# OpenRL-Lab/openrl

Measured on NVIDIA H100. Metric: env-steps/sec (collect+update), CartPole-v1 PPO, higher is better.
Workload: dtype f32 (nets, losses, Adam; the three 64x64 GEMM groups of the update run as split-fp16 wgmma MMAs with fp32 accumulation = fp32-class accuracy, the mode the 1e-4 parity tests run in), f64 (CartPole state)

## Files before the change

### include/openrl_b200.h

```cpp
#ifndef OPENRL_B200_H
#define OPENRL_B200_H

#include <stdint.h>

#ifdef __cplusplus
extern "C" {
#endif

#define ORL_ABI_VERSION 1

#define ORL_ERR_BAD_ARG 10001
#define ORL_ERR_UNSUPPORTED 10002

int orl_abi_version(void);
const char* orl_last_error(void);
int orl_device_sm_count(int* sm_count_out);

#define ORL_GAE_USE_GAE 1
#define ORL_GAE_PROPER_TIME_LIMITS 2
#define ORL_GAE_DENORM 4
#define ORL_GAE_NSTATS 8
#define ORL_GS_ADV_SUM 0
#define ORL_GS_ADV_SQSUM 1
#define ORL_GS_COUNT 2
#define ORL_GS_ADV_ACT_SUM 3
#define ORL_GS_ADV_ACT_SQSUM 4
#define ORL_GS_RET_SUM 5
#define ORL_GS_RET_SQSUM 6
#define ORL_GS_ACT_COUNT 7
int orl_gae(const float* rewards, float* value_preds, const float* masks,
            const float* bad_masks, const float* active_masks, const float* next_value,
            const float* vn_state, float* returns, float* advantages, double* stats,
            int T, int B, double gamma, double gae_lambda, int flags, void* stream);


#define ORL_HEAD_CATEGORICAL 0
#define ORL_HEAD_GAUSSIAN 1
#define ORL_HEAD_GAUSSIAN_WIDE 2
#define ORL_ENV_NONE 0
#define ORL_ENV_CARTPOLE 1
#define ORL_ENV_GRIDWORLD 2
#define ORL_ENV_MPE_SPREAD 3

int orl_env_reset(int env_kind, int n_envs, int n_agents, double* env_f64, uint64_t* env_u64,
                  int32_t* env_i32, const int32_t* env_table, int env_table_len,
                  uint64_t rng_seed, float* policy_obs_out, float* critic_obs_out, void* stream);

int orl_env_step(int env_kind, int n_envs, int n_agents, double* env_f64, uint64_t* env_u64,
                 int32_t* env_i32, const int32_t* env_table, int env_table_len, uint64_t rng_seed,
                 float* ep_return, int32_t* ep_length, double* episode_stats, const float* actions,
                 float* obs_out, float* rewards_out, float* dones_out, float* final_obs_out,
                 void* stream);

typedef struct OrlRolloutArgs {
    int32_t env_kind;
    int32_t n_envs;
    int32_t n_agents;
    int32_t episode_length;
    int32_t t_begin, t_end;
    int32_t obs_dim;
    int32_t critic_obs_dim;
    int32_t n_actions;
    int32_t activation_id;
    int32_t deterministic;
    int32_t env_table_len;
    const float* policy_params;
    float* policy_obs;
    float* critic_obs;
    float* actions;
    float* action_log_probs;
    float* rewards;
    float* masks;
    float* active_masks;
    const float* action_masks;
    const float* exp_noise;
    uint64_t rng_seed;
    uint64_t rng_step_base;
    uint64_t* rng_counter;
    double* env_f64;
    uint64_t* env_u64;
    int32_t* env_i32;
    const int32_t* env_table;
    float* ep_return;
    int32_t* ep_length;
    double* episode_stats;
    int32_t head_kind;
    int32_t rng_row_offset;
} OrlRolloutArgs;
int orl_rollout(const OrlRolloutArgs* args, void* stream);

int orl_critic_values(const float* critic_params, int obs_dim, int activation_id,
                      const float* obs, float* values, long long rows, void* stream);

int orl_host_insert(const float* staged, int n_envs, int n_agents, int obs_dim, float* policy_obs_next, float* rewards,
                    float* masks_next, float* active_masks_next, float* action_masks_next, int n_actions,
                    float* critic_obs_next, int critic_obs_dim, void* stream);
int orl_host_insert_wide_obs(const float* staged, int n_envs, int n_agents, int obs_dim, float* policy_obs_next, float* rewards,
                             float* masks_next, float* active_masks_next, float* action_masks_next, int n_actions,
                             float* critic_obs_next, int critic_obs_dim, void* stream);

int orl_policy_eval(const float* policy_params, int obs_dim, int n_actions, int activation_id, int head_kind,
                    const float* obs, const float* actions, const float* action_masks, float* log_probs,
                    float* entropy, long long rows, void* stream);


#define ORL_PPO_HUBER 1
#define ORL_PPO_CLIP_VALUE 2
#define ORL_PPO_VALUE_ACTIVE_MASKS 4
#define ORL_PPO_POLICY_ACTIVE_MASKS 8
#define ORL_PPO_VALUENORM 16
#define ORL_PPO_ADV_NORMALIZE 32
#define ORL_PPO_MAX_GRAD_NORM 64
#define ORL_PPO_A2C 256
#define ORL_PPO_DUAL_CLIP 512
#define ORL_PPO_TENSORCORE 128
#define ORL_PPO_TF32 ORL_PPO_TENSORCORE
#define ORL_PPO_JOINT_ACTION 1024

typedef struct OrlPpoArgs {
    int32_t obs_dim;
    int32_t critic_obs_dim;
    int32_t n_actions;
    int32_t activation_id;
    int32_t flags;
    int32_t grid_per_net;
    int64_t batch_rows;
    int64_t row_begin;
    int64_t total_rows;
    const int64_t* indices;
    const float* policy_obs;
    const float* critic_obs;
    const float* actions;
    const float* old_log_probs;
    const float* advantages;
    const float* value_preds;
    const float* returns;
    const float* active_masks;
    const float* action_masks;
    const double* gae_stats;
    const double* mb_stats;
    float* vn_state;
    float* policy_params;
    float* critic_params;
    float* policy_adam_m; float* policy_adam_v;
    float* critic_adam_m; float* critic_adam_v;
    int32_t* adam_steps;
    const float* lrs;
    float clip_param, entropy_coef, value_loss_coef, huber_delta, max_grad_norm;
    float adam_beta1, adam_beta2, adam_eps, weight_decay;
    float reserved0;
    double vn_beta;
    float* partials;
    float* folded;
    float* grads;
    float* train_info;
    int32_t head_kind;
    float dual_clip_coeff;
    int64_t norm_rows;
} OrlPpoArgs;
int orl_ppo_stride(int obs_dim, int critic_obs_dim, int n_actions);
int orl_ppo_grads_stride(int obs_dim, int critic_obs_dim, int n_actions);
int orl_net_param_count(int obs_dim, int n_out);
int orl_ppo_fwdbwd(const OrlPpoArgs* args, void* stream);
int orl_ppo_reduce(const OrlPpoArgs* args, void* stream);
int orl_ppo_apply(const OrlPpoArgs* args, void* stream);

#define ORL_PEER_MAX_WORLD 16
#define ORL_PEER_SMALL_MAX 16
typedef struct OrlPeerArgs {
    const uint64_t* peer_buffers;
    float* local_buffer;
    uint32_t* epochs;
    int32_t* error_flag;
    float* summed;
    int32_t world, rank;
    int32_t timeout_ms;
    int32_t reserved;
} OrlPeerArgs;
long long orl_ppo_peer_bucket_bytes(int obs_dim, int critic_obs_dim, int n_actions, int world);
int orl_ppo_reduce_peer(const OrlPpoArgs* args, const OrlPeerArgs* peer, void* stream);
int orl_ppo_apply_peer(const OrlPpoArgs* args, const OrlPeerArgs* peer, void* stream);
int orl_peer_sum_f64(const OrlPeerArgs* peer, int stride, double* data, int n, void* stream);
int orl_minibatch_stats(const int64_t* indices, int64_t batch_rows, const float* returns,
                        const float* active_masks, double* mb_stats_out, void* stream);


typedef struct OrlRnnArgs {
    int32_t env_kind, n_envs, n_agents, episode_length;
    int32_t t_begin, t_end;
    int32_t obs_dim, critic_obs_dim, n_actions, activation_id;
    int32_t deterministic, chunk_length;
    int32_t flags;
    int32_t env_table_len;
    int64_t n_chunks;
    const int64_t* chunk_ids;
    float* policy_params; float* critic_params;
    float* policy_obs; float* critic_obs;
    float* rnn_states; float* rnn_states_critic;
    float* actions; float* action_log_probs; float* rewards;
    float* masks; float* active_masks;
    float* value_preds; const float* returns; const float* advantages;
    const float* exp_noise;
    uint64_t rng_seed; uint64_t rng_step_base; uint64_t* rng_counter;
    double* env_f64; uint64_t* env_u64; int32_t* env_i32; const int32_t* env_table;
    float* ep_return; int32_t* ep_length; double* episode_stats;
    const double* gae_stats; const double* mb_stats; float* vn_state;
    float* tape;
    float* grads;
    int32_t grads_stride; int32_t reserved1;
    float* loss_acc;
    float* policy_adam_m; float* policy_adam_v; float* critic_adam_m; float* critic_adam_v;
    int32_t* adam_steps; const float* lrs;
    float clip_param, entropy_coef, value_loss_coef, huber_delta, max_grad_norm;
    float adam_beta1, adam_beta2, adam_eps, weight_decay, dual_clip_coeff;
    double vn_beta;
    float* train_info;
    int64_t norm_rows;
    int32_t rng_row_offset;
    int32_t row_begin, row_end;
    int32_t reserved2;
    const float* action_masks;
    int32_t head_kind;
    int32_t reserved3;
} OrlRnnArgs;
int orl_rnn_param_count(int obs_dim, int n_out);
int orl_rnn_param_count_head(int obs_dim, int n_out, int head_kind);
int orl_rnn_tape_width(void);
long long orl_rnn_workspace_floats(long long rows, int grads_stride);
long long orl_rnn_workspace_floats_for(long long rows, int grads_stride, int n_actions);
long long orl_rnn_workspace_floats_wide_obs(long long rows, int grads_stride, int n_actions, int obs_dim, int critic_obs_dim);
long long orl_rnn_workspace_floats_head(long long rows, int grads_stride, int n_actions, int obs_dim, int critic_obs_dim,
                                        int head_kind);
int orl_rnn_rollout(const OrlRnnArgs* args, void* stream);
int orl_rnn_act_rows(const OrlRnnArgs* args, void* stream);
int orl_host_insert_rnn(const float* staged, int n_envs, int n_agents, int obs_dim, float* policy_obs_next, float* rewards,
                        float* masks_next, float* active_masks_next, float* rnn_states_next, float* action_masks_next,
                        int n_actions, float* critic_obs_next, int critic_obs_dim, void* stream);
int orl_host_insert_rnn_wide(const float* staged, int n_envs, int n_agents, int obs_dim, float* policy_obs_next, float* rewards,
                             float* masks_next, float* active_masks_next, float* rnn_states_next, float* action_masks_next,
                             int n_actions, float* critic_obs_next, int critic_obs_dim, void* stream);
int orl_host_insert_rnn_wide_obs(const float* staged, int n_envs, int n_agents, int obs_dim, float* policy_obs_next, float* rewards,
                                 float* masks_next, float* active_masks_next, float* rnn_states_next, float* action_masks_next,
                                 int n_actions, float* critic_obs_next, int critic_obs_dim, void* stream);
int orl_rnn_critic(const OrlRnnArgs* args, void* stream);
int orl_rnn_fwdbwd(const OrlRnnArgs* args, void* stream);
int orl_rnn_apply(const OrlRnnArgs* args, void* stream);


#define ORL_ENV_GRIDWORLD_2P 4
#define ORL_SP_RANDOM 0
#define ORL_SP_LAST 1
typedef struct OrlSelfPlayArgs {
    OrlRolloutArgs rollout;
    const float* pool_params;
    const int32_t* pool_count;
    int32_t* pool_stats;
    int32_t pool_capacity, pool_stride, strategy, reserved;
} OrlSelfPlayArgs;
int orl_selfplay_reset(const OrlSelfPlayArgs* args, float* policy_obs_out, void* stream);
int orl_selfplay_rollout(const OrlSelfPlayArgs* args, void* stream);

int orl_share_param_count(int obs_dim, int n_actions);
int orl_share_param_count_head(int obs_dim, int n_actions, int head_kind);
int orl_share_tape_width(void);
long long orl_share_workspace_floats(long long rows, int obs_dim, int n_actions);
long long orl_share_workspace_floats_head(long long rows, int obs_dim, int n_actions, int head_kind);
int orl_share_rollout(const OrlRolloutArgs* args, void* stream);
int orl_share_values(const float* params, int obs_dim, int n_actions, int activation_id, const float* obs, float* values,
                     long long rows, void* stream);
int orl_share_fwdbwd(const OrlPpoArgs* args, void* stream);
int orl_share_apply(const OrlPpoArgs* args, void* stream);

#ifdef __cplusplus
}
#endif
#endif
```

### openrl_b200/algorithms/ppo.py

```python
import numpy as np
import torch
from .. import lib, parallel
from ..buffers.replay_data import ReplayData, chunk_row_indices, v3_row_indices


class PPOAlgorithm:
    def __init__(self, cfg, init_module, agent_num=1, device="cuda:0"):
        self.cfg = cfg
        self.algo_module = init_module
        self.agent_num = agent_num
        self.device = torch.device(device) if not isinstance(device, torch.device) else device
        self.world_size = parallel.world_size()
        self.ppo_epoch, self.num_mini_batch = cfg.ppo_epoch, cfg.num_mini_batch
        self.clip_param = cfg.clip_param
        self._lib = lib.load()
        pol, cri = init_module.models["policy"], init_module.models["critic"]
        self.d, self.dc, self.n = pol.obs_dim, cri.obs_dim, pol.n_actions
        self.stride = self._lib.orl_ppo_stride(self.d, self.dc, self.n)
        self.head_kind = pol.head_kind
        self.recurrent = bool(cfg.use_recurrent_policy or getattr(cfg, "use_naive_recurrent_policy", False))
        self.naive = bool(getattr(cfg, "use_naive_recurrent_policy", False)) and not cfg.use_recurrent_policy
        self.use_tensor_cores = (bool(getattr(cfg, "use_tensor_cores", True)) and bool(getattr(cfg, "use_tf32", True))
                                 and max(self.d, self.dc) <= 8 and self.n <= 8 and self.head_kind == lib.HEAD_CATEGORICAL
                                 and not self.recurrent)
        sm = torch.cuda.get_device_properties(self.device).multi_processor_count
        self.grid_per_net = max(1, sm if self.use_tensor_cores else sm // 2)
        dev = self.device
        self.partials = torch.zeros(2 * self.grid_per_net, self.stride, dtype=torch.float32, device=dev)
        self.folded, self.folded_sum = parallel.symmetric_buffer((2, self.stride), torch.float32, dev)
        self.peer = None
        if self.world_size > 1 and not self.recurrent and not bool(getattr(cfg, "use_share_model", False)):
            self.peer = parallel.PeerBucket.create(self._lib.orl_ppo_peer_bucket_bytes(self.d, self.dc, self.n, self.world_size),
                                                    self.stride, dev)
        self.grads_stride = self._lib.orl_ppo_grads_stride(self.d, self.dc, self.n)
        self.grads = torch.zeros(2, self.grads_stride, dtype=torch.float32, device=dev)
        self.train_info = torch.zeros(6, dtype=torch.float32, device=dev)
        self.lrs = torch.zeros(2, dtype=torch.float32, device=dev)
        self.mb_stats = torch.zeros(3, dtype=torch.float64, device=dev)
        self.flags = ((lib.PPO_HUBER if cfg.use_huber_loss else 0) | (lib.PPO_CLIP_VALUE if cfg.use_clipped_value_loss else 0)
                      | (lib.PPO_VALUE_ACTIVE_MASKS if cfg.use_value_active_masks else 0)
                      | (lib.PPO_POLICY_ACTIVE_MASKS if cfg.use_policy_active_masks else 0)
                      | (lib.PPO_VALUENORM if (cfg.use_valuenorm and cri.value_normalizer is not None) else 0)
                      | (lib.PPO_ADV_NORMALIZE if cfg.use_adv_normalize else 0)
                      | (lib.PPO_MAX_GRAD_NORM if cfg.use_max_grad_norm else 0))
        if self.use_tensor_cores:
            self.flags |= lib.PPO_TENSORCORE
        if getattr(cfg, "dual_clip_ppo", False):
            self.flags |= lib.PPO_DUAL_CLIP
        assert not (getattr(cfg, "use_popart", False) and cfg.use_valuenorm), \
            "self._use_popart and self._use_valuenorm can not be set True simultaneously"
        self.share = bool(getattr(init_module, "share_model", False))
        if self.share:
            if self.recurrent:
                raise NotImplementedError("use_share_model with recurrent policies is not built")
            self.use_tensor_cores = False
            self.flags &= ~lib.PPO_TENSORCORE
            self.share_total = int(self._lib.orl_share_param_count_head(self.d, self.n, self.head_kind))
            self.share_bucket = torch.zeros(((self.share_total + 3) & ~3) + 8, dtype=torch.float32, device=dev)
            self.share_grads = self.share_bucket[:(self.share_total + 3) & ~3]
            self.share_loss = self.share_bucket[(self.share_total + 3) & ~3:]
            self.share_ws = None
        for name in ("use_policy_vhead", "use_amp", "use_deepspeed"):
            if getattr(cfg, name, False):
                raise NotImplementedError(f"cfg.{name} is not built into the CUDA update yet (SURVEY.md §8f)")
        self.joint_action = bool(getattr(cfg, "use_joint_action_loss", False))
        if self.joint_action and (not cfg.use_recurrent_policy or self.share):
            raise NotImplementedError("use_joint_action_loss (JRPO) is built for the chunked recurrent update: it needs "
                                      "use_recurrent_policy and is not built with use_share_model or the feed-forward / "
                                      "naive-recurrent generators")
        if self.joint_action and self.n > 8:
            raise NotImplementedError("use_joint_action_loss (JRPO) is built for Discrete action spaces of up to 8 actions")
        if self.recurrent:
            gaussian_ok = bool(getattr(cfg, "use_recurrent_gaussian_head", False)) and (
                self.head_kind == lib.HEAD_GAUSSIAN
                or (self.head_kind == lib.HEAD_GAUSSIAN_WIDE and bool(getattr(cfg, "use_wide_recurrent_gaussian_head", False))))
            if self.head_kind != lib.HEAD_CATEGORICAL and not gaussian_ok:
                raise NotImplementedError("recurrent policies are built for Discrete action spaces")
            if gaussian_ok and self.joint_action:
                raise NotImplementedError("use_joint_action_loss (JRPO) is built for Discrete action spaces")
            self.chunk_length = cfg.episode_length if self.naive else cfg.data_chunk_length
            if not 1 <= self.chunk_length <= 32:
                raise NotImplementedError("the recurrent kernels take chunks of 1..32 steps (data_chunk_length, or episode_length "
                                          "with use_naive_recurrent_policy)")
            self.rnn_stride = (max(self._lib.orl_rnn_param_count_head(self.d, self.n, self.head_kind),
                                   self._lib.orl_rnn_param_count(self.dc, 1)) + 3) & ~3
            self.rnn_bucket = torch.zeros(2 * self.rnn_stride + 8, dtype=torch.float32, device=dev)
            self.rnn_grads = self.rnn_bucket[:2 * self.rnn_stride].view(2, self.rnn_stride)
            self.loss_acc = self.rnn_bucket[2 * self.rnn_stride:]
            self.tape = None
            if self.joint_action:
                self.joint_stats = torch.zeros(6, dtype=torch.float64, device=dev)
        self.gpu_launches = 0
        self.h2d_bytes = 0
        self.d2h_bytes = 0
        self._lrs_host = None

    def prep_rollout(self):
        pass

    def prep_training(self):
        pass

    def _common_args(self, a, rows):
        m = self.algo_module
        pol, cri = m.models["policy"], m.models["critic"]
        op, oc = m.optimizers["policy"], m.optimizers["critic"]
        cfg = self.cfg
        a.obs_dim, a.critic_obs_dim, a.n_actions, a.activation_id = self.d, self.dc, self.n, pol.activation_id
        a.policy_params, a.critic_params = lib.ptr(pol.flat_params), lib.ptr(cri.flat_params)
        a.policy_adam_m, a.policy_adam_v = lib.ptr(op.exp_avg), lib.ptr(op.exp_avg_sq)
        a.critic_adam_m, a.critic_adam_v = lib.ptr(oc.exp_avg), lib.ptr(oc.exp_avg_sq)
        a.adam_steps, a.lrs = lib.ptr(m.adam_steps), lib.ptr(self.lrs)
        a.clip_param, a.entropy_coef, a.value_loss_coef = cfg.clip_param, cfg.entropy_coef, cfg.value_loss_coef
        a.huber_delta, a.max_grad_norm = cfg.huber_delta, cfg.max_grad_norm
        g = op.param_groups[0]
        a.adam_beta1, a.adam_beta2, a.adam_eps, a.weight_decay = g["betas"][0], g["betas"][1], g["eps"], g["weight_decay"]
        a.dual_clip_coeff = float(getattr(cfg, "dual_clip_coeff", 3.0))
        vn = cri.value_normalizer
        a.vn_state = None if vn is None else lib.ptr(vn.state)
        a.vn_beta = 0.99999 if vn is None else vn.beta
        a.train_info = lib.ptr(self.train_info)
        a.norm_rows = int(rows) * self.world_size if self.world_size > 1 else 0
        return a

    def _args(self, buf, batch_rows, indices, row_begin):
        a = self._common_args(lib.OrlPpoArgs(), batch_rows)
        a.flags, a.grid_per_net = self.flags, self.grid_per_net
        a.head_kind = self.head_kind
        total = buf.episode_length * buf.n_rollout_threads * buf.num_agents
        a.batch_rows, a.row_begin, a.total_rows = int(batch_rows), int(row_begin), int(total)
        a.indices = lib.ptr(indices)
        a.policy_obs, a.critic_obs = lib.ptr(buf.policy_obs), lib.ptr(buf.critic_obs)
        a.actions, a.old_log_probs = lib.ptr(buf.actions), lib.ptr(buf.action_log_probs)
        a.advantages, a.value_preds, a.returns = lib.ptr(buf.advantages), lib.ptr(buf.value_preds), lib.ptr(buf.returns)
        a.active_masks = lib.ptr(buf.active_masks)
        a.action_masks = None if (buf.action_masks_trivial or buf.continuous) else lib.ptr(buf.action_masks)
        a.gae_stats = lib.ptr(buf.gae_stats)
        a.partials, a.folded, a.grads = lib.ptr(self.partials), lib.ptr(self.folded), lib.ptr(self.grads)
        return a

    def _share_update(self, buf, batch_rows, indices, row_begin, mb_stats):
        L, s = self._lib, lib.current_stream()
        need = int(L.orl_share_workspace_floats_head(int(batch_rows), self.d, self.n, self.head_kind))
        if self.share_ws is None or self.share_ws.numel() < need:
            self.share_ws = torch.empty(need, dtype=torch.float32, device=self.device)
        a = self._args(buf, batch_rows, indices, row_begin)
        a.mb_stats = lib.ptr(mb_stats)
        a.partials, a.grads, a.folded = lib.ptr(self.share_ws), lib.ptr(self.share_grads), lib.ptr(self.share_loss)
        lib.check(L.orl_share_fwdbwd(a, s), "orl_share_fwdbwd")
        parallel.allreduce_sum_(self.share_bucket)
        lib.check(L.orl_share_apply(a, s), "orl_share_apply")
        self.gpu_launches += 6

    def ppo_update(self, buf, batch_rows, indices=None, row_begin=0, mb_stats=None):
        L, s = self._lib, lib.current_stream()
        if mb_stats is None:
            lib.check(L.orl_minibatch_stats(lib.ptr(indices), int(batch_rows), lib.ptr(buf.returns),
                                            lib.ptr(buf.active_masks), lib.ptr(self.mb_stats), s), "orl_minibatch_stats")
            mb_stats = self.mb_stats
            self.gpu_launches += 1
            parallel.allreduce_sum_(mb_stats)
        if self.share:
            return self._share_update(buf, batch_rows, indices, row_begin, mb_stats)
        a = self._args(buf, batch_rows, indices, row_begin)
        a.mb_stats = lib.ptr(mb_stats)
        lib.check(L.orl_ppo_fwdbwd(a, s), "orl_ppo_fwdbwd")
        if self.peer is not None:
            lib.check(L.orl_ppo_reduce_peer(a, self.peer.args, s), "orl_ppo_reduce_peer")
            lib.check(L.orl_ppo_apply_peer(a, self.peer.args, s), "orl_ppo_apply_peer")
            self.gpu_launches += 3
            return
        lib.check(L.orl_ppo_reduce(a, s), "orl_ppo_reduce")
        summed = parallel.allreduce_sum_into(self.folded)
        a.folded = lib.ptr(summed)
        lib.check(L.orl_ppo_apply(a, s), "orl_ppo_apply")
        self.gpu_launches += 3

    def _rnn_args(self, buf, chunk_ids, mb_stats):
        a = self._common_args(lib.OrlRnnArgs(), int(chunk_ids.numel()) * self.chunk_length)
        a.n_envs, a.n_agents, a.episode_length = buf.n_rollout_threads, buf.num_agents, buf.episode_length
        a.chunk_length, a.flags = self.chunk_length, self.flags | (lib.PPO_JOINT_ACTION if self._joint(buf) else 0)
        a.n_chunks, a.chunk_ids = int(chunk_ids.numel()), lib.ptr(chunk_ids)
        a.policy_obs, a.critic_obs = lib.ptr(buf.policy_obs), lib.ptr(buf.critic_obs)
        a.rnn_states, a.rnn_states_critic = lib.ptr(buf.rnn_states), lib.ptr(buf.rnn_states_critic)
        a.actions, a.action_log_probs = lib.ptr(buf.actions), lib.ptr(buf.action_log_probs)
        a.masks, a.active_masks = lib.ptr(buf.masks), lib.ptr(buf.active_masks)
        a.action_masks = None if (buf.action_masks_trivial or buf.continuous) else lib.ptr(buf.action_masks)
        a.value_preds, a.returns, a.advantages = lib.ptr(buf.value_preds), lib.ptr(buf.returns), lib.ptr(buf.advantages)
        a.gae_stats, a.mb_stats = lib.ptr(buf.gae_stats), lib.ptr(mb_stats)
        a.tape, a.grads, a.grads_stride, a.loss_acc = lib.ptr(self.tape), lib.ptr(self.rnn_grads), self.rnn_stride, lib.ptr(self.loss_acc)
        a.head_kind = self.head_kind
        return a

    def _joint(self, buf):
        return self.joint_action and buf.num_agents > 1

    def _joint_mb_stats(self, buf, ids):
        T, A = buf.episode_length, buf.num_agents
        s = lib.current_stream()
        for k, every in ((0, False), (3, True)):
            bi = v3_row_indices(ids, self.chunk_length, T, A, buf.n_rollout_threads * A, all_agents=every)
            lib.check(self._lib.orl_minibatch_stats(lib.ptr(bi), int(bi.numel()), lib.ptr(buf.returns), lib.ptr(buf.active_masks),
                                                    lib.ptr(self.joint_stats[k:k + 3]), s), "orl_minibatch_stats")
        self.gpu_launches += 2
        parallel.allreduce_sum_(self.joint_stats)
        return self.joint_stats

    def _train_recurrent(self, buf):
        cfg = self.cfg
        T, B = buf.episode_length, buf.n_rollout_threads * buf.num_agents
        joint = self._joint(buf)
        total, L = (T * buf.n_rollout_threads if joint else T * B), (T if self.naive else cfg.data_chunk_length)
        if total < L:
            raise AssertionError(f"PPO requires the number of processes ({buf.n_rollout_threads}) * episode length ({T}) "
                                 f"{'' if joint else '* agents '}to be greater than or equal to the data chunk length ({L}).")
        data_chunks = total // L
        mbc = data_chunks // self.num_mini_batch
        rows = mbc * L
        tape_rows = rows * buf.num_agents if joint else rows
        need = int(self._lib.orl_rnn_workspace_floats_head(tape_rows, self.rnn_stride, self.n, self.d, self.dc, self.head_kind))
        if self.tape is None or self.tape.numel() < need:
            self.tape = torch.empty(need, dtype=torch.float32, device=self.device)
        whole = self.num_mini_batch == 1 and rows == total and not joint
        s, Lb = lib.current_stream(), self._lib
        for _ in range(self.ppo_epoch):
            if cfg.parity_mode:
                perm = torch.randperm(data_chunks).to(self.device, non_blocking=True)
                self.h2d_bytes += data_chunks * 8
            else:
                perm = torch.randperm(data_chunks, device=self.device)
            for i in range(self.num_mini_batch):
                ids = perm[i * mbc:(i + 1) * mbc].contiguous()
                if joint:
                    mb_stats = self._joint_mb_stats(buf, ids)
                elif whole:
                    mb_stats = buf.gae_stats[5:8]
                else:
                    bi = chunk_row_indices(ids, L, T, B)
                    lib.check(Lb.orl_minibatch_stats(lib.ptr(bi), int(rows), lib.ptr(buf.returns), lib.ptr(buf.active_masks),
                                                     lib.ptr(self.mb_stats), s), "orl_minibatch_stats")
                    mb_stats = self.mb_stats
                    self.gpu_launches += 1
                    parallel.allreduce_sum_(mb_stats)
                a = self._rnn_args(buf, ids, mb_stats)
                lib.check(Lb.orl_rnn_fwdbwd(a, s), "orl_rnn_fwdbwd")
                parallel.allreduce_sum_(self.rnn_bucket)
                lib.check(Lb.orl_rnn_apply(a, s), "orl_rnn_apply")
                self.gpu_launches += 9

    def train(self, buffer, turn_on=True):
        if not isinstance(buffer, ReplayData):
            buffer = ReplayData.from_host(buffer, self.cfg, self.algo_module.get_critic_value_normalizer(), device=self.device)
            self.h2d_bytes += buffer.h2d_bytes
        self.train_async(buffer)
        return self.read_train_info()

    def read_train_info(self):
        num_updates = self.ppo_epoch * self.num_mini_batch
        info = (self.train_info / num_updates).cpu().numpy()
        self.d2h_bytes += info.nbytes
        if self.peer is not None and not (info == info).all():
            self.peer.check()
        keys = ["value_loss", "critic_grad_norm", "policy_loss", "dist_entropy", "actor_grad_norm", "ratio"]
        return {k: float(v) for k, v in zip(keys, info)}

    def sync_lrs(self):
        m = self.algo_module
        lrs = (m.optimizers["policy"].param_groups[0]["lr"], m.optimizers["critic"].param_groups[0]["lr"])
        if lrs != self._lrs_host:
            self.lrs.copy_(torch.tensor(lrs, dtype=torch.float32), non_blocking=True)
            self._lrs_host = lrs
            self.h2d_bytes += 8

    def train_async(self, buffer):
        buf = buffer
        if not torch.cuda.is_current_stream_capturing():
            self.sync_lrs()
        self.train_info.zero_()
        if not getattr(buf, "returns_ready", True):
            buf.compute_returns(None, self.algo_module.get_critic_value_normalizer())
            self.gpu_launches += 1
        if not getattr(buf, "stats_global", False):
            if self.peer is not None and buf.gae_stats.numel() <= 16:
                lib.check(self._lib.orl_peer_sum_f64(self.peer.args, self.stride, lib.ptr(buf.gae_stats), buf.gae_stats.numel(),
                                                     lib.current_stream()), "orl_peer_sum_f64")
                self.gpu_launches += 1
            else:
                parallel.allreduce_sum_(buf.gae_stats)
            buf.stats_global = True
        if self.recurrent:
            return self._train_recurrent(buf)
        total = buf.episode_length * buf.n_rollout_threads * buf.num_agents
        mb = total // self.num_mini_batch
        whole = self.num_mini_batch == 1
        for _ in range(self.ppo_epoch):
            if self.cfg.parity_mode:
                perm = torch.randperm(total).to(self.device, non_blocking=True)
                self.h2d_bytes += total * 8
            elif whole:
                perm = None
            else:
                perm = torch.randperm(total, device=self.device)
            for i in range(self.num_mini_batch):
                if whole:
                    self.ppo_update(buf, mb, perm, 0, mb_stats=buf.gae_stats[5:8])
                else:
                    self.ppo_update(buf, mb, perm[i * mb:(i + 1) * mb])
```

### openrl_b200/csrc/orl_common.cuh

```cuda
#pragma once
#include <cuda_runtime.h>
#include <stdint.h>
#include <stdio.h>

#include "openrl_b200.h"

namespace orl {

void set_last_error(const char* fmt, ...);
int check_cuda(cudaError_t e, const char* what);
int sm_count();
int bump_rng_counter(uint64_t* counter, int steps, cudaStream_t st);
int allow_dynamic_smem(const void* kernel, size_t smem_bytes, bool max_carveout = false);
template <typename K>
int allow_dynamic_smem(K* kernel, size_t smem_bytes, bool max_carveout = false) {
    return allow_dynamic_smem(reinterpret_cast<const void*>(kernel), smem_bytes, max_carveout);
}

struct TapeJob { int p_off, M, q_off, N, out_off; };
constexpr int TAPE_MAX_GEMM_JOBS = 6, TAPE_MAX_COL_JOBS = 15;
struct TapeJobs { TapeJob gemm[TAPE_MAX_GEMM_JOBS]; TapeJob col[TAPE_MAX_COL_JOBS]; int n_gemm, n_col; };
constexpr int TAPE_ROW_BLOCK = 1024;
int reduce_tape(const float* tape, int tape_width, long long rows, const TapeJobs& jobs, float* partials, int stride, int total,
                float* grads, cudaStream_t st);

#define ORL_CHECK_ARG(cond, msg)                                   \
    do {                                                           \
        if (!(cond)) {                                             \
            orl::set_last_error("%s: bad argument: %s", __func__, msg); \
            return ORL_ERR_BAD_ARG;                                \
        }                                                          \
    } while (0)

#define ORL_LAUNCH_CHECK(what) \
    do { int _e = orl::check_cuda(cudaGetLastError(), what); if (_e) return _e; } while (0)

__device__ __forceinline__ float warp_sum(float v) {
#pragma unroll
    for (int o = 16; o > 0; o >>= 1) v += __shfl_xor_sync(0xffffffffu, v, o);
    return v;
}
__device__ __forceinline__ double warp_sum(double v) {
#pragma unroll
    for (int o = 16; o > 0; o >>= 1) v += __shfl_xor_sync(0xffffffffu, v, o);
    return v;
}

struct VnScalars { float mean, std, var; };
__device__ __forceinline__ VnScalars vn_mean_std(const float* __restrict__ vn_state) {
    const float rm = vn_state[0], rms = vn_state[1], db = vn_state[2];
    const float d = fmaxf(db, 1e-5f);
    const float m = __fdiv_rn(rm, d);
    const float msq = __fdiv_rn(rms, d);
    float var = __fsub_rn(msq, __fmul_rn(m, m));
    var = fmaxf(var, 1e-2f);
    VnScalars s; s.mean = m; s.var = var; s.std = __fsqrt_rn(var);
    return s;
}

}
```

### openrl_b200/csrc/orl_mlp.cuh

```cuda
#pragma once
#include "orl_common.cuh"

namespace orl {

constexpr int H = 64;
constexpr int LDA = 68;
constexpr int MAX_OUT = 8;
constexpr int MAX_OUT_WIDE = 64;
constexpr int OBS_PANEL = 64;
constexpr int LDX_PANEL = OBS_PANEL + 4;
constexpr int MAX_OBS_WIDE = 256;
constexpr float LN_EPS = 1e-5f;

struct NetOffsets {
    int d, n;
    int w1, b1, g1, be1, w3, b3, g3, be3, wh, bh, ls, total;
};
__host__ __device__ inline NetOffsets net_offsets(int d, int n, int gaussian = 0) {
    NetOffsets o; o.d = d; o.n = n;
    int p = 0;
    o.w1 = p; p += H * d;  o.b1 = p; p += H;  o.g1 = p; p += H;  o.be1 = p; p += H;
    o.w3 = p; p += H * H;  o.b3 = p; p += H;  o.g3 = p; p += H;  o.be3 = p; p += H;
    o.wh = p; p += n * H;  o.bh = p; p += n;
    o.ls = p; if (gaussian) p += n;
    o.total = p;
    return o;
}
struct FoldOffsets { int g1, db1, g3, db3, gh, dbh, dls, total; };
__host__ __device__ inline FoldOffsets fold_offsets(int d, int n) {
    FoldOffsets o; int p = 0;
    o.g1 = p; p += H * d;  o.db1 = p; p += H;  o.g3 = p; p += H * H;  o.db3 = p; p += H;
    o.gh = p; p += n * H;  o.dbh = p; p += n;  o.dls = p; p += n;  o.total = p;
    return o;
}

__device__ __forceinline__ float folded_w3(const float* P, const NetOffsets& o, int j, int k) { return P[o.w3 + j * H + k] * P[o.g1 + k]; }
__device__ __forceinline__ float folded_b3(const float* P, const NetOffsets& o, int j) {
    float s = P[o.b3 + j];
    for (int k = 0; k < H; ++k) s = fmaf(P[o.w3 + j * H + k], P[o.be1 + k], s);
    return s;
}
__device__ __forceinline__ float folded_wh(const float* P, const NetOffsets& o, int j, int k) {
    return j < o.n ? P[o.wh + j * H + k] * P[o.g3 + k] : 0.f;
}
__device__ __forceinline__ float folded_bh(const float* P, const NetOffsets& o, int j) {
    float s = 0.f;
    if (j < o.n) {
        s = P[o.bh + j];
        for (int k = 0; k < H; ++k) s = fmaf(P[o.wh + j * H + k], P[o.be3 + k], s);
    }
    return s;
}
__device__ __forceinline__ float unfolded_grad(const float* P, const NetOffsets& po, const FoldOffsets& fo, const float* f, int i) {
    if (i < po.b1) return f[fo.g1 + (i - po.w1)];
    if (i < po.g1) return f[fo.db1 + (i - po.b1)];
    if (i < po.be1) {
        const int k = i - po.g1; float s = 0.f;
        for (int j = 0; j < H; ++j) s = fmaf(P[po.w3 + j * H + k], f[fo.g3 + j * H + k], s);
        return s;
    }
    if (i < po.w3) {
        const int k = i - po.be1; float s = 0.f;
        for (int j = 0; j < H; ++j) s = fmaf(P[po.w3 + j * H + k], f[fo.db3 + j], s);
        return s;
    }
    if (i < po.b3) {
        const int j = (i - po.w3) / H, k = (i - po.w3) % H;
        return fmaf(f[fo.g3 + j * H + k], P[po.g1 + k], f[fo.db3 + j] * P[po.be1 + k]);
    }
    if (i < po.g3) return f[fo.db3 + (i - po.b3)];
    if (i < po.be3) {
        const int k = i - po.g3; float s = 0.f;
        for (int j = 0; j < po.n; ++j) s = fmaf(P[po.wh + j * H + k], f[fo.gh + j * H + k], s);
        return s;
    }
    if (i < po.wh) {
        const int k = i - po.be3; float s = 0.f;
        for (int j = 0; j < po.n; ++j) s = fmaf(P[po.wh + j * H + k], f[fo.dbh + j], s);
        return s;
    }
    if (i < po.bh) {
        const int j = (i - po.wh) / H, k = (i - po.wh) % H;
        return fmaf(f[fo.gh + j * H + k], P[po.g3 + k], f[fo.dbh + j] * P[po.be3 + k]);
    }
    if (i < po.ls) return f[fo.dbh + (i - po.bh)];
    return f[fo.dls + (i - po.ls)];
}

__host__ __device__ inline int pad4(int x) { return (x + 3) & ~3; }

struct SmemWeights {
    float* w1t;
    float* b1;
    float* w3t;
    float* w3n;
    float* b3f;
    float* whf;
    float* wht;
    float* bhf;
};
template <int NB = MAX_OUT>
__host__ __device__ inline int smem_weights_floats(int d, bool backward) {
    const int head = NB == MAX_OUT ? MAX_OUT * H : (backward ? H * H : 0) + H * H;
    return pad4(d) * H + H + H * H + (backward ? H * H : 0) + H + head + NB;
}
template <int NB = MAX_OUT>
__device__ inline SmemWeights carve_weights(float*& p, int d, bool backward) {
    static_assert(NB == MAX_OUT || NB == MAX_OUT_WIDE, "head width bound");
    SmemWeights w;
    w.w1t = p; p += pad4(d) * H;
    w.b1 = p; p += H;
    w.w3t = p; p += H * H;
    w.w3n = backward ? p : nullptr; if (backward) p += H * H;
    w.b3f = p; p += H;
    if (NB == MAX_OUT) {
        w.whf = p; p += MAX_OUT * H;
        w.wht = nullptr;
    } else {
        w.whf = backward ? p : nullptr; if (backward) p += H * H;
        w.wht = p; p += H * H;
    }
    w.bhf = p; p += NB;
    return w;
}

template <int NT, int NB = MAX_OUT, bool PANELS = false>
__device__ inline void load_weights_folded(const SmemWeights& w, const float* __restrict__ params, int d, int n,
                                           bool backward) {
    const NetOffsets o = net_offsets(d, n);
    const int tid = threadIdx.x, dp = pad4(d);
    if (!PANELS) {
        for (int i = tid; i < dp * H; i += NT) {
            const int k = i / H, j = i % H;
            w.w1t[i] = (k < d) ? params[o.w1 + j * d + k] : 0.f;
        }
    }
    for (int i = tid; i < H; i += NT) w.b1[i] = params[o.b1 + i];
    for (int i = tid; i < H * H; i += NT) {
        const int j = i / H, k = i % H;
        const float v = folded_w3(params, o, j, k);
        w.w3t[k * H + j] = v;
        if (backward) w.w3n[i] = v;
    }
    if (NB == MAX_OUT) {
        for (int i = tid; i < MAX_OUT * H; i += NT) w.whf[i] = folded_wh(params, o, i / H, i % H);
    } else {
        for (int i = tid; i < H * H; i += NT) {
            const int j = i / H, k = i % H;
            const float v = folded_wh(params, o, j, k);
            w.wht[k * H + j] = v;
            if (backward) w.whf[i] = v;
        }
    }
    for (int j = tid; j < H; j += NT) w.b3f[j] = folded_b3(params, o, j);
    for (int j = tid; j < NB; j += NT) w.bhf[j] = folded_bh(params, o, j);
    __syncthreads();
}

__device__ __forceinline__ float half_warp_sum(float v) {
    v += __shfl_xor_sync(0xffffffffu, v, 8);
    v += __shfl_xor_sync(0xffffffffu, v, 4);
    v += __shfl_xor_sync(0xffffffffu, v, 2);
    v += __shfl_xor_sync(0xffffffffu, v, 1);
    return v;
}

template <int RPT, int TY>
__device__ __forceinline__ void gemm_tile(const float* __restrict__ A, int lda, const float* __restrict__ Bt, int K,
                                          float (&acc)[RPT][4], int tx, int ty) {
    const float* a_base = A + ty * lda;
    const float* b_base = Bt + 4 * tx;
#pragma unroll 2
    for (int k0 = 0; k0 < K; k0 += 4) {
        const float4 b0 = *reinterpret_cast<const float4*>(b_base + (k0 + 0) * H);
        const float4 b1 = *reinterpret_cast<const float4*>(b_base + (k0 + 1) * H);
        const float4 b2 = *reinterpret_cast<const float4*>(b_base + (k0 + 2) * H);
        const float4 b3 = *reinterpret_cast<const float4*>(b_base + (k0 + 3) * H);
#pragma unroll
        for (int i = 0; i < RPT; ++i) {
            const float4 a = *reinterpret_cast<const float4*>(a_base + i * TY * lda + k0);
            acc[i][0] = fmaf(a.x, b0.x, acc[i][0]); acc[i][1] = fmaf(a.x, b0.y, acc[i][1]);
            acc[i][2] = fmaf(a.x, b0.z, acc[i][2]); acc[i][3] = fmaf(a.x, b0.w, acc[i][3]);
            acc[i][0] = fmaf(a.y, b1.x, acc[i][0]); acc[i][1] = fmaf(a.y, b1.y, acc[i][1]);
            acc[i][2] = fmaf(a.y, b1.z, acc[i][2]); acc[i][3] = fmaf(a.y, b1.w, acc[i][3]);
            acc[i][0] = fmaf(a.z, b2.x, acc[i][0]); acc[i][1] = fmaf(a.z, b2.y, acc[i][1]);
            acc[i][2] = fmaf(a.z, b2.z, acc[i][2]); acc[i][3] = fmaf(a.z, b2.w, acc[i][3]);
            acc[i][0] = fmaf(a.w, b3.x, acc[i][0]); acc[i][1] = fmaf(a.w, b3.y, acc[i][1]);
            acc[i][2] = fmaf(a.w, b3.z, acc[i][2]); acc[i][3] = fmaf(a.w, b3.w, acc[i][3]);
        }
    }
}

__device__ __forceinline__ float act_fwd(float z, int activation_id) {
    switch (activation_id) {
        case 0: return tanhf(z);
        case 1: return fmaxf(z, 0.f);
        case 2: return z > 0.f ? z : 0.01f * z;
        default: return z > 0.f ? z : expm1f(z);
    }
}
__device__ __forceinline__ float act_bwd(float a, bool pos, int activation_id) {
    switch (activation_id) {
        case 0: return 1.f - a * a;
        case 1: return pos ? 1.f : 0.f;
        case 2: return pos ? 1.f : 0.01f;
        default: return pos ? 1.f : a + 1.f;
    }
}

template <int RPT>
__device__ __forceinline__ void layernorm_rows(float (&acc)[RPT][4], float (&mu)[RPT], float (&rstd)[RPT]) {
#pragma unroll
    for (int i = 0; i < RPT; ++i) {
        float s = (acc[i][0] + acc[i][1]) + (acc[i][2] + acc[i][3]);
        s = half_warp_sum(s);
        const float m = s * (1.f / H);
        const float d0 = acc[i][0] - m, d1 = acc[i][1] - m, d2 = acc[i][2] - m, d3 = acc[i][3] - m;
        float v = (d0 * d0 + d1 * d1) + (d2 * d2 + d3 * d3);
        v = half_warp_sum(v);
        const float r = 1.0f / sqrtf(v * (1.f / H) + LN_EPS);
        acc[i][0] = d0 * r; acc[i][1] = d1 * r; acc[i][2] = d2 * r; acc[i][3] = d3 * r;
        mu[i] = m; rstd[i] = r;
    }
}

template <int RPT>
__device__ __forceinline__ void layernorm_bwd_rows(float (&dn)[RPT][4], const float (&nrm)[RPT][4],
                                                   const float (&rstd)[RPT]) {
#pragma unroll
    for (int i = 0; i < RPT; ++i) {
        float s1 = (dn[i][0] + dn[i][1]) + (dn[i][2] + dn[i][3]);
        float s2 = (dn[i][0] * nrm[i][0] + dn[i][1] * nrm[i][1]) + (dn[i][2] * nrm[i][2] + dn[i][3] * nrm[i][3]);
        s1 = half_warp_sum(s1) * (1.f / H);
        s2 = half_warp_sum(s2) * (1.f / H);
#pragma unroll
        for (int c = 0; c < 4; ++c) dn[i][c] = rstd[i] * (dn[i][c] - s1 - nrm[i][c] * s2);
    }
}

template <int RPT, int TY>
__device__ __forceinline__ void store_tile(float* __restrict__ S, const float (&acc)[RPT][4], int tx, int ty) {
#pragma unroll
    for (int i = 0; i < RPT; ++i)
        *reinterpret_cast<float4*>(S + (ty + TY * i) * LDA + 4 * tx) =
            make_float4(acc[i][0], acc[i][1], acc[i][2], acc[i][3]);
}
template <int RPT, int TY>
__device__ __forceinline__ void load_tile(const float* __restrict__ S, float (&acc)[RPT][4], int tx, int ty) {
#pragma unroll
    for (int i = 0; i < RPT; ++i) {
        const float4 v = *reinterpret_cast<const float4*>(S + (ty + TY * i) * LDA + 4 * tx);
        acc[i][0] = v.x; acc[i][1] = v.y; acc[i][2] = v.z; acc[i][3] = v.w;
    }
}

template <int M, int NT, bool KEEP>
__device__ __forceinline__ void trunk_from_z1(const SmemWeights& w, float (&acc)[M / (NT / 16)][4], int activation_id,
                                              float* __restrict__ N1s, float* __restrict__ N3s,
                                              float (&mu1)[M / (NT / 16)], float (&rstd1)[M / (NT / 16)],
                                              float (&rstd3)[M / (NT / 16)], unsigned& posmask) {
    constexpr int TY = NT / 16, RPT = M / TY;
    const int tx = threadIdx.x & 15, ty = threadIdx.x >> 4;
    unsigned pm = 0;
#pragma unroll
    for (int i = 0; i < RPT; ++i)
#pragma unroll
        for (int c = 0; c < 4; ++c) {
            if (KEEP && acc[i][c] > 0.f) pm |= 1u << (i * 4 + c);
            acc[i][c] = act_fwd(acc[i][c], activation_id);
        }
    posmask = pm;
    layernorm_rows<RPT>(acc, mu1, rstd1);
    store_tile<RPT, TY>(N1s, acc, tx, ty);
    __syncthreads();
    {
        const float4 b = *reinterpret_cast<const float4*>(w.b3f + 4 * tx);
#pragma unroll
        for (int i = 0; i < RPT; ++i) { acc[i][0] = b.x; acc[i][1] = b.y; acc[i][2] = b.z; acc[i][3] = b.w; }
    }
    gemm_tile<RPT, TY>(N1s, LDA, w.w3t, H, acc, tx, ty);
    float mu3[RPT];
    layernorm_rows<RPT>(acc, mu3, rstd3);
    store_tile<RPT, TY>(N3s, acc, tx, ty);
}

template <int M, int NT, bool KEEP>
__device__ __forceinline__ void trunk_forward(const SmemWeights& w, const float* __restrict__ Xs, int ldx, int d,
                                              int activation_id, float* __restrict__ N1s, float* __restrict__ N3s,
                                              float (&mu1)[M / (NT / 16)], float (&rstd1)[M / (NT / 16)],
                                              float (&rstd3)[M / (NT / 16)], unsigned& posmask) {
    constexpr int TY = NT / 16, RPT = M / TY;
    const int tx = threadIdx.x & 15, ty = threadIdx.x >> 4;
    float acc[RPT][4];
    {
        const float4 b = *reinterpret_cast<const float4*>(w.b1 + 4 * tx);
#pragma unroll
        for (int i = 0; i < RPT; ++i) { acc[i][0] = b.x; acc[i][1] = b.y; acc[i][2] = b.z; acc[i][3] = b.w; }
    }
    gemm_tile<RPT, TY>(Xs, ldx, w.w1t, pad4(d), acc, tx, ty);
    trunk_from_z1<M, NT, KEEP>(w, acc, activation_id, N1s, N3s, mu1, rstd1, rstd3, posmask);
}


template <int M, int NT, typename RowPtr>
__device__ __forceinline__ void stage_obs_panel(float* __restrict__ Xs, int d, int p, RowPtr&& row) {
    for (int i = threadIdx.x; i < M * LDX_PANEL; i += NT) {
        const int r = i / LDX_PANEL, k = i % LDX_PANEL, c = OBS_PANEL * p + k;
        const float* src = row(r);
        Xs[i] = (src != nullptr && k < OBS_PANEL && c < d) ? src[c] : 0.f;
    }
}

template <int M, int NT, typename RowPtr>
__device__ __forceinline__ void fc1_panels(const SmemWeights& w, const float* __restrict__ W1, int d, float* __restrict__ Xs,
                                           RowPtr&& row, float (&acc)[M / (NT / 16)][4]) {
    constexpr int TY = NT / 16, RPT = M / TY;
    const int tx = threadIdx.x & 15, ty = threadIdx.x >> 4;
    {
        const float4 b = *reinterpret_cast<const float4*>(w.b1 + 4 * tx);
#pragma unroll
        for (int i = 0; i < RPT; ++i) { acc[i][0] = b.x; acc[i][1] = b.y; acc[i][2] = b.z; acc[i][3] = b.w; }
    }
    const int P = (d + OBS_PANEL - 1) / OBS_PANEL;
    for (int p = 0; p < P; ++p) {
        __syncthreads();
        for (int i = threadIdx.x; i < OBS_PANEL * H; i += NT) {
            const int k = 8 * (i / (8 * H)) + i % 8, j = (i / 8) % H, c = OBS_PANEL * p + k;
            w.w1t[k * H + j] = c < d ? W1[j * d + c] : 0.f;
        }
        stage_obs_panel<M, NT>(Xs, d, p, row);
        __syncthreads();
        gemm_tile<RPT, TY>(Xs, LDX_PANEL, w.w1t, min(OBS_PANEL, pad4(d - OBS_PANEL * p)), acc, tx, ty);
    }
}

template <int M, int NT>
__device__ __forceinline__ void head_dots(const SmemWeights& w, const float* __restrict__ N3s, int n,
                                          float (&out)[MAX_OUT]) {
    constexpr int PPR = NT / M;
    static_assert(PPR == 1 || PPR == 2 || PPR == 4 || PPR == 8 || PPR == 16, "threads per row");
    const int row = threadIdx.x / PPR, part = threadIdx.x % PPR;
#pragma unroll
    for (int j = 0; j < MAX_OUT; ++j) out[j] = 0.f;
    for (int q = part; q < H / 4; q += PPR) {
        const float4 a = *reinterpret_cast<const float4*>(N3s + row * LDA + 4 * q);
#pragma unroll
        for (int j = 0; j < MAX_OUT; ++j) {
            if (j < n) {
                const float4 ww = *reinterpret_cast<const float4*>(w.whf + j * H + 4 * q);
                out[j] = fmaf(a.x, ww.x, fmaf(a.y, ww.y, fmaf(a.z, ww.z, fmaf(a.w, ww.w, out[j]))));
            }
        }
    }
#pragma unroll
    for (int j = 0; j < MAX_OUT; ++j) {
        if (j < n) {
#pragma unroll
            for (int o = PPR / 2; o > 0; o >>= 1) out[j] += __shfl_xor_sync(0xffffffffu, out[j], o);
            out[j] += w.bhf[j];
        }
    }
}

template <int M, int NT>
__device__ __forceinline__ void head_tile(const SmemWeights& w, const float* __restrict__ N3s, float* __restrict__ Ls) {
    constexpr int TY = NT / 16, RPT = M / TY;
    const int tx = threadIdx.x & 15, ty = threadIdx.x >> 4;
    float acc[RPT][4];
    const float4 b = *reinterpret_cast<const float4*>(w.bhf + 4 * tx);
#pragma unroll
    for (int i = 0; i < RPT; ++i) { acc[i][0] = b.x; acc[i][1] = b.y; acc[i][2] = b.z; acc[i][3] = b.w; }
    gemm_tile<RPT, TY>(N3s, LDA, w.wht, H, acc, tx, ty);
    store_tile<RPT, TY>(Ls, acc, tx, ty);
}

}
```

### openrl_b200/csrc/orl_ppo.cu

```cuda
#include <algorithm>

#include "orl_adam.cuh"

namespace {
using namespace orl;

constexpr int P_M = 128;
constexpr int P_NT = 256;
constexpr int P_TY = P_NT / 16, P_RPT = P_M / P_TY;
constexpr int DLW = 8;
constexpr int N_LOSS = 8;

__host__ __device__ inline int ppo_stride(int obs_dim, int critic_obs_dim, int n_actions) {
    const int a = orl::fold_offsets(obs_dim, n_actions).total, b = orl::fold_offsets(critic_obs_dim, 1).total;
    return ((a > b ? a : b) + N_LOSS + 3) & ~3;
}

__host__ __device__ inline int ppo_grads_stride(int obs_dim, int critic_obs_dim, int n_actions) {
    const int a = orl::net_offsets(obs_dim, n_actions, 1).total, b = orl::net_offsets(critic_obs_dim, 1).total;
    return ((a > b ? a : b) + 3) & ~3;
}

struct WgMap { int jb, kb, mg, MG; bool active; };
__device__ __forceinline__ WgMap wg_map(int JB, int KB) {
    WgMap m;
    const int nb = JB * KB;
    m.MG = P_NT / nb;
    const int tid = threadIdx.x;
    m.active = tid < nb * m.MG;
    const int b = tid % nb;
    m.mg = tid / nb;
    m.jb = b / KB;
    m.kb = b % KB;
    return m;
}
__device__ __forceinline__ void wgrad_acc(const float* __restrict__ P, int ldp, const float* __restrict__ Q, int ldq,
                                          const WgMap& mp, float (&g)[4][4], float (&db)[4]) {
    if (!mp.active) return;
    const float* pp = P + 4 * mp.jb;
    const float* qq = Q + 4 * mp.kb;
    const bool bias = mp.kb == 0;
#pragma unroll 4
    for (int m = mp.mg; m < P_M; m += mp.MG) {
        const float4 p = *reinterpret_cast<const float4*>(pp + m * ldp);
        const float4 q = *reinterpret_cast<const float4*>(qq + m * ldq);
        g[0][0] = fmaf(p.x, q.x, g[0][0]); g[0][1] = fmaf(p.x, q.y, g[0][1]); g[0][2] = fmaf(p.x, q.z, g[0][2]); g[0][3] = fmaf(p.x, q.w, g[0][3]);
        g[1][0] = fmaf(p.y, q.x, g[1][0]); g[1][1] = fmaf(p.y, q.y, g[1][1]); g[1][2] = fmaf(p.y, q.z, g[1][2]); g[1][3] = fmaf(p.y, q.w, g[1][3]);
        g[2][0] = fmaf(p.z, q.x, g[2][0]); g[2][1] = fmaf(p.z, q.y, g[2][1]); g[2][2] = fmaf(p.z, q.z, g[2][2]); g[2][3] = fmaf(p.z, q.w, g[2][3]);
        g[3][0] = fmaf(p.w, q.x, g[3][0]); g[3][1] = fmaf(p.w, q.y, g[3][1]); g[3][2] = fmaf(p.w, q.z, g[3][2]); g[3][3] = fmaf(p.w, q.w, g[3][3]);
        if (bias) { db[0] += p.x; db[1] += p.y; db[2] += p.z; db[3] += p.w; }
    }
}

__device__ __forceinline__ void wgrad_flush(float* __restrict__ scratch, const WgMap& mp, int JB, int KB,
                                            const float (&g)[4][4], const float (&db)[4], int jdim, int kdim,
                                            float* __restrict__ out, float* __restrict__ out_b) {
    const int W = 4 * KB, R = 4 * JB;
    __syncthreads();
    if (mp.active) {
        float* s = scratch + (size_t)mp.mg * (R * W + R);
#pragma unroll
        for (int a = 0; a < 4; ++a)
#pragma unroll
            for (int b = 0; b < 4; ++b) s[(4 * mp.jb + a) * W + 4 * mp.kb + b] = g[a][b];
        if (mp.kb == 0) {
#pragma unroll
            for (int a = 0; a < 4; ++a) s[R * W + 4 * mp.jb + a] = db[a];
        }
    }
    __syncthreads();
    for (int i = threadIdx.x; i < R * W + R; i += P_NT) {
        float v = 0.f;
        for (int g2 = 0; g2 < mp.MG; ++g2) v += scratch[(size_t)g2 * (R * W + R) + i];
        if (i < R * W) {
            const int j = i / W, k = i % W;
            if (j < jdim && k < kdim) out[j * kdim + k] = v;
        } else {
            const int j = i - R * W;
            if (j < jdim) out_b[j] = v;
        }
    }
}


template <bool POLICY, int NB = MAX_OUT, bool PANELS = false, bool GAUSS = false>
__device__ __forceinline__ void ppo_net_pass(const OrlPpoArgs& a, float* smem, int cta, int G) {
    constexpr bool WIDE = NB == MAX_OUT_WIDE;
    static_assert(POLICY || !WIDE, "the critic's head is one value");
    static_assert(WIDE || !GAUSS, "GAUSS is the wide DiagGaussian head");
    static_assert(P_NT % MAX_OUT_WIDE == 0, "whole row groups of the dimension-parallel loss");
    const int d = POLICY ? a.obs_dim : a.critic_obs_dim;
    const int n = POLICY ? a.n_actions : 1;
    const float* params = POLICY ? a.policy_params : a.critic_params;
    const float* obs = POLICY ? a.policy_obs : a.critic_obs;
    const int dp = PANELS ? OBS_PANEL : pad4(d), ldx = dp + 4;
    const int tid = threadIdx.x, tx = tid & 15, ty = tid >> 4;

    float* p = smem;
    SmemWeights w = carve_weights<NB>(p, PANELS ? OBS_PANEL : d, true);
    float* Xs = p;  p += P_M * ldx;
    float* N1s = p; p += P_M * LDA;
    float* N3s = p; p += P_M * LDA;
    float* DZs = p; p += P_M * LDA;
    float* DLs = p; if (!WIDE) p += P_M * DLW;
    float* row_a = p; p += P_M;
    float* row_b = p; p += P_M;
    float* row_c = p; p += P_M;
    float* row_act = p; p += P_M;
    float* red = p; p += 32;
    long long* row_idx = reinterpret_cast<long long*>(p); p += 2 * P_M;

    load_weights_folded<P_NT, NB, PANELS>(w, params, d, n, true);

    const bool pol_masks = a.flags & ORL_PPO_POLICY_ACTIVE_MASKS, val_masks = a.flags & ORL_PPO_VALUE_ACTIVE_MASKS;
    const MbConsts mb = mb_consts(a);

    const WgMap map3 = wg_map(16, 16);
    const WgMap map1 = wg_map(16, dp / 4);
    const int JBH = WIDE ? (n + 3) / 4 : n > 4 ? 2 : 1;
    const WgMap maph = wg_map(JBH, 16);
    float g3[4][4] = {}, g1[4][4] = {}, gh[4][4] = {}, db3[4] = {}, db1[4] = {}, dbh[4] = {};
    const bool gaussian = POLICY && !WIDE && a.head_kind == ORL_HEAD_GAUSSIAN;
    float dls_acc[MAX_OUT] = {};
    float dls_wide = 0.f;
    float loss0 = 0.f, loss1 = 0.f, loss2 = 0.f;

    const int n_panels = (d + OBS_PANEL - 1) / OBS_PANEL;
    float* g1_part = nullptr;
    if constexpr (PANELS)
        g1_part = a.partials + (size_t)((POLICY ? 0 : G) + cta) * ppo_stride(a.obs_dim, a.critic_obs_dim, a.n_actions) +
                  fold_offsets(d, n).g1;
    auto g1_at = [&](int pnl, int r, int c) -> float* {
        return g1_part + (4 * map1.jb + r) * d + OBS_PANEL * pnl + 4 * map1.kb + c;
    };
    if constexpr (PANELS) {
        for (int pnl = 0; pnl < n_panels; ++pnl)
#pragma unroll
            for (int r = 0; r < 4; ++r)
#pragma unroll
                for (int c = 0; c < 4; ++c)
                    if (OBS_PANEL * pnl + 4 * map1.kb + c < d) *g1_at(pnl, r, c) = 0.f;
    }
    auto obs_row = [&](int r) -> const float* { return row_idx[r] >= 0 ? obs + row_idx[r] * d : nullptr; };

    const long long n_tiles = (a.batch_rows + P_M - 1) / P_M;
    for (long long tile = cta; tile < n_tiles; tile += G) {
        const long long r0 = tile * P_M;
        const int rows_here = (int)min((long long)P_M, a.batch_rows - r0);
        if (tid < P_M) {
            long long gi = -1;
            if (tid < rows_here) gi = a.indices ? a.indices[r0 + tid] : a.row_begin + r0 + tid;
            row_idx[tid] = gi;
            if (gi >= 0) {
                if (POLICY) { row_a[tid] = a.actions[gi]; row_b[tid] = a.old_log_probs[gi]; row_c[tid] = a.advantages[gi]; }
                else { row_a[tid] = a.value_preds[gi]; row_b[tid] = a.returns[gi]; }
                row_act[tid] = a.active_masks[gi];
            }
        }
        __syncthreads();
        float mu1[P_RPT], rstd1[P_RPT], rstd3[P_RPT];
        unsigned posmask;
        float acc[P_RPT][4];
        if constexpr (PANELS) {
            fc1_panels<P_M, P_NT>(w, params + net_offsets(d, n).w1, d, Xs, obs_row, acc);
            trunk_from_z1<P_M, P_NT, true>(w, acc, a.activation_id, N1s, N3s, mu1, rstd1, rstd3, posmask);
        } else {
            for (int i = tid; i < P_M * ldx; i += P_NT) {
                const int r = i / ldx, k = i % ldx;
                const long long gi = row_idx[r];
                Xs[i] = (gi >= 0 && k < d) ? obs[gi * d + k] : 0.f;
            }
            __syncthreads();
            trunk_forward<P_M, P_NT, true>(w, Xs, ldx, d, a.activation_id, N1s, N3s, mu1, rstd1, rstd3, posmask);
        }
        __syncthreads();
        if constexpr (WIDE) {
            head_tile<P_M, P_NT>(w, N3s, DZs);
            __syncthreads();
            if constexpr (GAUSS) {
                constexpr int RG = P_NT / MAX_OUT_WIDE;
                const int j = tid % MAX_OUT_WIDE;
                if (j < pad4(n)) {
                    const float ls = j < n ? params[net_offsets(d, n, 1).ls + j] : 0.f, std = expf(ls), var = std * std;
                    const float ent_j = gaussian_entropy(ls);
                    for (int r = tid / MAX_OUT_WIDE; r < P_M; r += RG) {
                        float* x = DZs + r * LDA + j;
                        if (r < rows_here && j < n) {
                            const long long gi = row_idx[r];
                            const float active = row_act[r];
                            const float wrow = mb.weight(pol_masks, active);
                            const float went_row = pol_masks ? active * mb.inv_act : mb.inv_rows / (float)n;
                            const float diff = a.actions[gi * n + j] - *x;
                            const PgTerm pg = pg_term(gaussian_log_prob(diff, std, ls), a.old_log_probs[gi * n + j],
                                                      apply_adv_norm(mb.adv, row_c[r]), a.clip_param, a.flags, a.dual_clip_coeff);
                            loss0 += pg.loss * wrow;
                            loss1 += ent_j * went_row;
                            loss2 += pg.ratio / (float)n;
                            const float dlp = pg.dlogp * wrow;
                            *x = dlp * diff / var;
                            dls_wide += dlp * (diff * diff / var - 1.0f) - a.entropy_coef * went_row;
                        } else {
                            *x = 0.f;
                        }
                    }
                }
            } else if (tid < P_M) {
                float* x = DZs + tid * LDA;
                if (tid < rows_here) {
                    const long long gi = row_idx[tid];
                    const float wrow = mb.weight(pol_masks, row_act[tid]);
                    const CatRow c = wide_categorical_row(a, x, n, a.action_masks ? a.action_masks + gi * n : nullptr, (int)row_a[tid],
                                                          row_b[tid], apply_adv_norm(mb.adv, row_c[tid]), wrow);
                    loss0 += c.loss * wrow;
                    loss1 += c.ent * wrow;
                    loss2 += c.ratio;
                } else {
                    for (int j = 0; j < pad4(n); ++j) x[j] = 0.f;
                }
            }
            __syncthreads();
#pragma unroll
            for (int i = 0; i < P_RPT; ++i) { acc[i][0] = acc[i][1] = acc[i][2] = acc[i][3] = 0.f; }
            gemm_tile<P_RPT, P_TY>(DZs, LDA, w.whf, pad4(n), acc, tx, ty);
            wgrad_acc(DZs, LDA, N3s, LDA, maph, gh, dbh);
            {
                float nrm[P_RPT][4];
                load_tile<P_RPT, P_TY>(N3s, nrm, tx, ty);
                layernorm_bwd_rows<P_RPT>(acc, nrm, rstd3);
            }
            __syncthreads();
            store_tile<P_RPT, P_TY>(DZs, acc, tx, ty);
            __syncthreads();
        } else {
            float out[MAX_OUT];
            head_dots<P_M, P_NT>(w, N3s, n, out);
            {
                constexpr int PPR = P_NT / P_M;
                const int row = tid / PPR;
                if (tid % PPR == 0) {
                    float dl[DLW];
#pragma unroll
                    for (int j = 0; j < DLW; ++j) dl[j] = 0.f;
                    if (row < rows_here) {
                        const float active = row_act[row];
                        if (POLICY && gaussian) {
                            const long long gi = row_idx[row];
                            const float went_row = pol_masks ? active * mb.inv_act : mb.inv_rows / (float)n;
                            gaussian_row(a, out, n, params + net_offsets(d, n, 1).ls, a.actions + gi * n, a.old_log_probs + gi * n,
                                         apply_adv_norm(mb.adv, row_c[row]), mb.weight(pol_masks, active), went_row, dl, dls_acc,
                                         loss0, loss1, loss2);
                        } else if (POLICY) {
                            const long long gi = row_idx[row];
                            const float wrow = mb.weight(pol_masks, active);
                            const CatRow c = categorical_row(a, out, n, a.action_masks ? a.action_masks + gi * n : nullptr, (int)row_a[row],
                                                             row_b[row], apply_adv_norm(mb.adv, row_c[row]), wrow, dl);
                            loss0 += c.loss * wrow;
                            loss1 += c.ent * wrow;
                            loss2 += c.ratio;
                        } else {
                            const float ret = row_b[row];
                            const float target = (a.flags & ORL_PPO_VALUENORM) ? (ret - mb.vn_mean) / mb.vn_std : ret;
                            const ValueTerm vt = value_term(out[0], row_a[row], target, a.clip_param, a.huber_delta, a.flags);
                            const float wrow = mb.weight(val_masks, active);
                            loss0 += vt.loss * wrow;
                            dl[0] = a.value_loss_coef * wrow * vt.dv;
                        }
                    }
                    *reinterpret_cast<float4*>(DLs + row * DLW) = make_float4(dl[0], dl[1], dl[2], dl[3]);
                    *reinterpret_cast<float4*>(DLs + row * DLW + 4) = make_float4(dl[4], dl[5], dl[6], dl[7]);
                }
            }
            __syncthreads();

#pragma unroll
            for (int i = 0; i < P_RPT; ++i) { acc[i][0] = acc[i][1] = acc[i][2] = acc[i][3] = 0.f; }
            for (int j = 0; j < n; ++j) {
                const float4 wv = *reinterpret_cast<const float4*>(w.whf + j * H + 4 * tx);
#pragma unroll
                for (int i = 0; i < P_RPT; ++i) {
                    const float dlv = DLs[(ty + P_TY * i) * DLW + j];
                    acc[i][0] = fmaf(dlv, wv.x, acc[i][0]); acc[i][1] = fmaf(dlv, wv.y, acc[i][1]);
                    acc[i][2] = fmaf(dlv, wv.z, acc[i][2]); acc[i][3] = fmaf(dlv, wv.w, acc[i][3]);
                }
            }
            {
                float nrm[P_RPT][4];
                load_tile<P_RPT, P_TY>(N3s, nrm, tx, ty);
                layernorm_bwd_rows<P_RPT>(acc, nrm, rstd3);
            }
            store_tile<P_RPT, P_TY>(DZs, acc, tx, ty);
            wgrad_acc(DLs, DLW, N3s, LDA, maph, gh, dbh);
            __syncthreads();
        }

        wgrad_acc(DZs, LDA, N1s, LDA, map3, g3, db3);
#pragma unroll
        for (int i = 0; i < P_RPT; ++i) { acc[i][0] = acc[i][1] = acc[i][2] = acc[i][3] = 0.f; }
        gemm_tile<P_RPT, P_TY>(DZs, LDA, w.w3n, H, acc, tx, ty);
        {
            float nrm[P_RPT][4];
            load_tile<P_RPT, P_TY>(N1s, nrm, tx, ty);
            layernorm_bwd_rows<P_RPT>(acc, nrm, rstd1);
#pragma unroll
            for (int i = 0; i < P_RPT; ++i) {
                const float stdv = 1.0f / rstd1[i];
#pragma unroll
                for (int c = 0; c < 4; ++c) {
                    const float aval = fmaf(nrm[i][c], stdv, mu1[i]);
                    acc[i][c] *= act_bwd(aval, (posmask >> (i * 4 + c)) & 1u, a.activation_id);
                }
            }
        }
        __syncthreads();
        store_tile<P_RPT, P_TY>(DZs, acc, tx, ty);
        __syncthreads();
        if constexpr (PANELS) {
            for (int pnl = n_panels - 1; pnl >= 0; --pnl) {
                if (pnl != n_panels - 1) {
                    stage_obs_panel<P_M, P_NT>(Xs, d, pnl, obs_row);
                    __syncthreads();
                }
                float gp[4][4] = {}, dbp[4] = {};
                wgrad_acc(DZs, LDA, Xs, LDX_PANEL, map1, gp, dbp);
#pragma unroll
                for (int r = 0; r < 4; ++r) {
                    if (pnl == 0) db1[r] += dbp[r];
#pragma unroll
                    for (int c = 0; c < 4; ++c)
                        if (OBS_PANEL * pnl + 4 * map1.kb + c < d) *g1_at(pnl, r, c) += gp[r][c];
                }
                __syncthreads();
            }
        } else {
            wgrad_acc(DZs, LDA, Xs, ldx, map1, g1, db1);
            __syncthreads();
        }
    }

    const int stride = ppo_stride(a.obs_dim, a.critic_obs_dim, a.n_actions);
    float* part = a.partials + (size_t)((POLICY ? 0 : G) + cta) * stride;
    const FoldOffsets fo = fold_offsets(d, n);
    float* scratch = N1s;
    if constexpr (PANELS) {
        if (map1.kb == 0) {
#pragma unroll
            for (int r = 0; r < 4; ++r) part[fo.db1 + 4 * map1.jb + r] = db1[r];
        }
    } else {
        wgrad_flush(scratch, map1, 16, dp / 4, g1, db1, H, d, part + fo.g1, part + fo.db1);
    }
    wgrad_flush(scratch, map3, 16, 16, g3, db3, H, H, part + fo.g3, part + fo.db3);
    wgrad_flush(scratch, maph, JBH, 16, gh, dbh, n, H, part + fo.gh, part + fo.dbh);
    __syncthreads();
    if (GAUSS) {
        scratch[tid] = dls_wide;
        __syncthreads();
        if (tid < n) {
            float sv = 0.f;
            for (int g2 = 0; g2 < P_NT / MAX_OUT_WIDE; ++g2) sv += scratch[g2 * MAX_OUT_WIDE + tid];
            part[fo.dls + tid] = sv;
        }
        __syncthreads();
    } else if (WIDE) {
        if (tid < n) part[fo.dls + tid] = 0.f;
    } else if (POLICY) {
        const int lane = tid & 31, warp = tid >> 5;
#pragma unroll
        for (int j = 0; j < MAX_OUT; ++j) {
            const float sv = warp_sum(dls_acc[j]);
            if (lane == 0) scratch[j * 8 + warp] = sv;
        }
        __syncthreads();
        if (tid < n) {
            float sv = 0.f;
            for (int wv = 0; wv < P_NT / 32; ++wv) sv += scratch[tid * 8 + wv];
            part[fo.dls + tid] = sv;
        }
        __syncthreads();
    } else if (tid < n) {
        part[fo.dls + tid] = 0.f;
    }
    {
        float v[3] = {loss0, loss1, loss2};
        const int lane = tid & 31, warp = tid >> 5;
#pragma unroll
        for (int k = 0; k < 3; ++k) {
            const float s = warp_sum(v[k]);
            if (lane == 0) red[k * 8 + warp] = s;
        }
        __syncthreads();
        if (tid < N_LOSS) {
            float s = 0.f;
            if (tid < 3) for (int wv = 0; wv < P_NT / 32; ++wv) s += red[tid * 8 + wv];
            part[stride - N_LOSS + tid] = s;
        }
    }
}

template <int NB, bool PANELS_POLICY, bool PANELS_CRITIC>
__global__ void __launch_bounds__(P_NT, 1) ppo_fwdbwd_kernel(const OrlPpoArgs a) {
    extern __shared__ __align__(16) float smem[];
    const int G = a.grid_per_net;
    if ((int)blockIdx.x < G) ppo_net_pass<true, NB, PANELS_POLICY>(a, smem, blockIdx.x, G);
    else ppo_net_pass<false, MAX_OUT, PANELS_CRITIC>(a, smem, blockIdx.x - G, G);
}

template <bool PANELS_POLICY, bool PANELS_CRITIC>
__global__ void __launch_bounds__(P_NT, 1) ppo_fwdbwd_gaussian_wide_kernel(const OrlPpoArgs a) {
    extern __shared__ __align__(16) float smem[];
    const int G = a.grid_per_net;
    if ((int)blockIdx.x < G) ppo_net_pass<true, MAX_OUT_WIDE, PANELS_POLICY, true>(a, smem, blockIdx.x, G);
    else ppo_net_pass<false, MAX_OUT, PANELS_CRITIC>(a, smem, blockIdx.x - G, G);
}

constexpr int RED_W = 8, RED_NT = 32 * RED_W;
__device__ __forceinline__ float reduce_partials(const float* __restrict__ partials, int net, int G, int stride, int el,
                                                 float (*part)[32]) {
    const int lane = threadIdx.x & 31, w = threadIdx.x >> 5;
    float s0 = 0.f, s1 = 0.f;
    if (el < stride) {
        const float* p = partials + (size_t)net * G * stride + el;
        int g = w;
#pragma unroll 4
        for (; g + RED_W < G; g += 2 * RED_W) { s0 += p[(size_t)g * stride]; s1 += p[(size_t)(g + RED_W) * stride]; }
        if (g < G) s0 += p[(size_t)g * stride];
    }
    part[w][lane] = s0 + s1;
    __syncthreads();
    float t = 0.f;
    if (w == 0) {
#pragma unroll
        for (int k = 0; k < RED_W; ++k) t += part[k][lane];
    }
    return t;
}

__global__ void __launch_bounds__(RED_NT) ppo_reduce_kernel(const float* __restrict__ partials, float* __restrict__ folded, int G, int stride) {
    __shared__ float part[RED_W][32];
    const int net = blockIdx.y, el = blockIdx.x * 32 + (threadIdx.x & 31);
    const float s = reduce_partials(partials, net, G, stride, el, part);
    if (threadIdx.x < 32 && el < stride) folded[(size_t)net * stride + el] = s;
}

__global__ void __launch_bounds__(RED_NT) ppo_reduce_peer_kernel(const float* __restrict__ partials, const OrlPeerArgs pa, int G, int stride) {
    __shared__ float part[RED_W][32];
    const int net = blockIdx.y, el = blockIdx.x * 32 + (threadIdx.x & 31);
    const float s = reduce_partials(partials, net, G, stride, el, part);
    if (threadIdx.x < 32 && el < stride) {
        const size_t off = ((size_t)(pa.epochs[net] & 1u) * pa.world + pa.rank) * 2u * stride + (size_t)net * stride + el;
        for (int q = 0; q < pa.world; ++q) reinterpret_cast<float*>(pa.peer_buffers[q])[off] = s;
    }
}

__device__ __forceinline__ void st_release_sys(uint32_t* p, uint32_t v) {
    asm volatile("st.release.sys.global.u32 [%0], %1;" ::"l"(p), "r"(v) : "memory");
}
__device__ __forceinline__ uint32_t ld_acquire_sys(const uint32_t* p) {
    uint32_t v;
    asm volatile("ld.acquire.sys.global.u32 %0, [%1];" : "=r"(v) : "l"(p) : "memory");
    return v;
}
__device__ __forceinline__ float4 ld_peer4(const float* p) {
    float4 v;
    asm volatile("ld.relaxed.sys.global.v4.f32 {%0,%1,%2,%3}, [%4];" : "=f"(v.x), "=f"(v.y), "=f"(v.z), "=f"(v.w) : "l"(p) : "memory");
    return v;
}
__device__ __forceinline__ uint64_t global_ns() {
    uint64_t t;
    asm volatile("mov.u64 %0, %globaltimer;" : "=l"(t));
    return t;
}

__host__ __device__ __forceinline__ size_t peer_flag_word(int world, int stride) { return (size_t)4 * world * stride; }

__device__ __forceinline__ void peer_handshake(const OrlPeerArgs& pa, int slot, uint32_t e, size_t flag_word) {
    const int tid = threadIdx.x, W = pa.world;
    if (tid < W) {
        __threadfence_system();
        uint32_t* remote = reinterpret_cast<uint32_t*>(pa.peer_buffers[tid]) + flag_word + slot * ORL_PEER_MAX_WORLD + pa.rank;
        st_release_sys(remote, e);
        const uint32_t* mine = reinterpret_cast<const uint32_t*>(pa.peer_buffers[pa.rank]) + flag_word + slot * ORL_PEER_MAX_WORLD + tid;
        const uint64_t t0 = global_ns();
        unsigned spins = 0;
        while ((int32_t)(ld_acquire_sys(mine) - e) < 0) {
            if ((++spins & 1023u) == 0 && global_ns() - t0 > (uint64_t)pa.timeout_ms * 1000000ull) {
                atomicExch(pa.error_flag, 1 + tid);
                break;
            }
        }
        __threadfence_system();
    }
    __syncthreads();
}

__device__ const float* peer_gather(const OrlPeerArgs& pa, int net, int stride) {
    const int tid = threadIdx.x, W = pa.world;
    const uint32_t e = pa.epochs[net] + 1u;
    peer_handshake(pa, net, e, peer_flag_word(W, stride));
    const float* base = pa.local_buffer + (size_t)((e - 1u) & 1u) * W * 2u * stride + (size_t)net * stride;
    float* out = pa.summed + (size_t)net * stride;
    for (int i = tid * 4; i < stride; i += blockDim.x * 4) {
        float4 s = make_float4(0.f, 0.f, 0.f, 0.f);
        for (int q0 = 0; q0 < W; q0 += 8) {
            float4 v[8];
#pragma unroll
            for (int q = 0; q < 8; ++q)
                if (q0 + q < W) v[q] = ld_peer4(base + (size_t)(q0 + q) * 2u * stride + i);
#pragma unroll
            for (int q = 0; q < 8; ++q)
                if (q0 + q < W) { s.x += v[q].x; s.y += v[q].y; s.z += v[q].z; s.w += v[q].w; }
        }
        *reinterpret_cast<float4*>(out + i) = s;
    }
    __syncthreads();
    return out;
}

__global__ void __launch_bounds__(64) peer_sum_f64_kernel(const OrlPeerArgs pa, double* __restrict__ data, int n, int stride) {
    const int tid = threadIdx.x, W = pa.world;
    const uint32_t e = pa.epochs[2] + 1u;
    const size_t flag_word = peer_flag_word(W, stride);
    const size_t small_byte = flag_word * 4 + (size_t)3 * ORL_PEER_MAX_WORLD * 4 + (size_t)((e - 1u) & 1u) * ORL_PEER_SMALL_MAX * 8;
    double* mine = reinterpret_cast<double*>(reinterpret_cast<char*>(pa.peer_buffers[pa.rank]) + small_byte);
    if (tid < n) mine[tid] = data[tid];
    __syncthreads();
    peer_handshake(pa, 2, e, flag_word);
    if (tid < n) {
        double s = 0.0;
        for (int q = 0; q < W; ++q) {
            double v;
            asm volatile("ld.relaxed.sys.global.f64 %0, [%1];" : "=d"(v)
                         : "l"(reinterpret_cast<const double*>(reinterpret_cast<const char*>(pa.peer_buffers[q]) + small_byte) + tid) : "memory");
            s += v;
        }
        data[tid] = s;
    }
    if (tid == 0) pa.epochs[2] = e;
}

template <bool PEER>
__global__ void __launch_bounds__(1024) ppo_apply_kernel(const OrlPpoArgs a, const OrlPeerArgs pa) {
    const int net = blockIdx.x;
    const int d = net == 0 ? a.obs_dim : a.critic_obs_dim;
    const int n = net == 0 ? a.n_actions : 1;
    const int stride = ppo_stride(a.obs_dim, a.critic_obs_dim, a.n_actions);
    const NetOffsets po = net_offsets(d, n, net == 0 && a.head_kind == ORL_HEAD_GAUSSIAN);
    const FoldOffsets fo = fold_offsets(d, n);
    float* params = net == 0 ? a.policy_params : a.critic_params;
    float* am = net == 0 ? a.policy_adam_m : a.critic_adam_m;
    float* av = net == 0 ? a.policy_adam_v : a.critic_adam_v;
    float* grads = a.grads + (size_t)net * ppo_grads_stride(a.obs_dim, a.critic_obs_dim, a.n_actions);
    const int tid = threadIdx.x;
    const float* f = PEER ? peer_gather(pa, net, stride) : a.folded + (size_t)net * stride;

    float sq = 0.f;
    for (int i = tid; i < po.total; i += blockDim.x) {
        const float g = unfolded_grad(params, po, fo, f, i);
        grads[i] = g;
        sq = fmaf(g, g, sq);
    }
    const float norm = block_l2_norm(sq);
    adam_step(a, net, params, am, av, grads, po.total, clip_factor(a, norm));
    if (tid == 0) {
        if (PEER) {
            pa.epochs[net] += 1u;
            if (*reinterpret_cast<volatile int32_t*>(pa.error_flag) != 0) a.train_info[net == 0 ? 2 : 0] = __int_as_float(0x7fc00000);
        }
        const float* ls = f + stride - N_LOSS;
        if (net == 0) add_policy_info(a, ls, norm);
        else add_value_info(a, ls[0], norm);
    }
}

__global__ void minibatch_stats_kernel(const int64_t* __restrict__ idx, int64_t rows, const float* __restrict__ returns,
                                       const float* __restrict__ active, double* __restrict__ out) {
    double s0 = 0, s1 = 0, s2 = 0;
    for (int64_t i = blockIdx.x * (int64_t)blockDim.x + threadIdx.x; i < rows; i += (int64_t)gridDim.x * blockDim.x) {
        const int64_t g = idx[i];
        const double r = returns[g];
        s0 += r; s1 += r * r; s2 += active[g];
    }
    __shared__ double red[3][8];
    const int lane = threadIdx.x & 31, warp = threadIdx.x >> 5;
    s0 = warp_sum(s0); s1 = warp_sum(s1); s2 = warp_sum(s2);
    if (lane == 0) { red[0][warp] = s0; red[1][warp] = s1; red[2][warp] = s2; }
    __syncthreads();
    if (threadIdx.x < 3) {
        double t = 0;
        for (int wv = 0; wv < (int)(blockDim.x >> 5); ++wv) t += red[threadIdx.x][wv];
        atomicAdd(out + threadIdx.x, t);
    }
}

size_t fwdbwd_smem_bytes(int d, int dc) {
    const int dm = std::max(d, dc);
    const int ldx = orl::pad4(dm) + 4;
    const size_t floats = orl::smem_weights_floats(dm, true) + (size_t)P_M * ldx + 3 * (size_t)P_M * orl::LDA +
                          (size_t)P_M * DLW + 4 * P_M + 32 + 4 * P_M  + 16;
    return floats * sizeof(float);
}
size_t fwdbwd_wide_smem_bytes(int d, int dc) {
    const size_t rest = (size_t)4 * P_M + 32 + 4 * P_M + 16;
    const size_t pol = orl::smem_weights_floats<orl::MAX_OUT_WIDE>(d, true) + (size_t)P_M * (orl::pad4(d) + 4) + 3 * (size_t)P_M * orl::LDA + rest;
    const size_t cri = orl::smem_weights_floats(dc, true) + (size_t)P_M * (orl::pad4(dc) + 4) + 3 * (size_t)P_M * orl::LDA + (size_t)P_M * DLW + rest;
    return std::max(pol, cri) * sizeof(float);
}

OrlPpoArgs apply_args(const OrlPpoArgs& a) {
    OrlPpoArgs b = a;
    if (b.head_kind == ORL_HEAD_GAUSSIAN_WIDE) b.head_kind = ORL_HEAD_GAUSSIAN;
    return b;
}

int check_ppo_args(const OrlPpoArgs& a) {
    ORL_CHECK_ARG(a.obs_dim > 0 && a.obs_dim <= orl::MAX_OBS_WIDE && a.critic_obs_dim > 0 && a.critic_obs_dim <= orl::MAX_OBS_WIDE,
                  "obs dims must be in 1..256");
    ORL_CHECK_ARG(a.n_actions > 0 && a.n_actions <= orl::MAX_OUT_WIDE, "n_actions must be in 1..64");
    ORL_CHECK_ARG(a.n_actions <= orl::MAX_OUT || a.head_kind == ORL_HEAD_CATEGORICAL || a.head_kind == ORL_HEAD_GAUSSIAN_WIDE,
                  "n_actions must be in 1..8 for Gaussian heads (1..64 for Categorical heads)");
    ORL_CHECK_ARG(a.activation_id >= 0 && a.activation_id <= 3, "activation_id");
    ORL_CHECK_ARG(a.grid_per_net > 0, "grid_per_net");
    ORL_CHECK_ARG(a.batch_rows > 0, "batch_rows");
    ORL_CHECK_ARG(a.policy_params && a.critic_params && a.partials && a.folded && a.grads && a.train_info, "null buffer");
    return 0;
}

}

namespace orl {
int ppo_stride_host(int obs_dim, int critic_obs_dim, int n_actions) { return ppo_stride(obs_dim, critic_obs_dim, n_actions); }
int launch_ppo_fwdbwd_tc(const OrlPpoArgs& a, cudaStream_t st);
}

extern "C" int orl_ppo_stride(int obs_dim, int critic_obs_dim, int n_actions) {
    return ppo_stride(obs_dim, critic_obs_dim, n_actions);
}

extern "C" int orl_ppo_grads_stride(int obs_dim, int critic_obs_dim, int n_actions) {
    return ppo_grads_stride(obs_dim, critic_obs_dim, n_actions);
}

extern "C" int orl_net_param_count(int obs_dim, int n_out) { return orl::net_offsets(obs_dim, n_out).total; }

extern "C" int orl_ppo_fwdbwd(const OrlPpoArgs* args, void* stream) {
    ORL_CHECK_ARG(args, "args");
    const OrlPpoArgs& a = *args;
    if (int e = check_ppo_args(a)) return e;
    ORL_CHECK_ARG(a.policy_obs && a.critic_obs && a.actions && a.old_log_probs && a.advantages && a.value_preds &&
                      a.returns && a.active_masks && a.gae_stats && a.mb_stats, "null rollout buffer");
    ORL_CHECK_ARG(!(a.flags & ORL_PPO_VALUENORM) || a.vn_state, "vn_state required with VALUENORM");
    ORL_CHECK_ARG(a.indices || (a.row_begin >= 0 && a.row_begin + a.batch_rows <= a.total_rows), "row range");
    ORL_CHECK_ARG(a.head_kind == ORL_HEAD_CATEGORICAL || a.head_kind == ORL_HEAD_GAUSSIAN || a.head_kind == ORL_HEAD_GAUSSIAN_WIDE,
                  "head_kind");
    if (a.flags & ORL_PPO_TF32) {
        ORL_CHECK_ARG(a.head_kind != ORL_HEAD_GAUSSIAN_WIDE, "ORL_PPO_TENSORCORE: ORL_HEAD_GAUSSIAN_WIDE is not supported");
        ORL_CHECK_ARG(a.n_actions <= orl::MAX_OUT, "ORL_PPO_TENSORCORE: n_actions must be in 1..8");
        ORL_CHECK_ARG(a.obs_dim <= orl::OBS_PANEL && a.critic_obs_dim <= orl::OBS_PANEL, "ORL_PPO_TENSORCORE: obs dims must be in 1..64");
        if (a.head_kind != ORL_HEAD_CATEGORICAL) {
            orl::set_last_error("orl_ppo_fwdbwd: ORL_PPO_TENSORCORE supports categorical heads only");
            return ORL_ERR_UNSUPPORTED;
        }
        return orl::launch_ppo_fwdbwd_tc(a, reinterpret_cast<cudaStream_t>(stream));
    }
    const bool wide = a.n_actions > orl::MAX_OUT;
    const int ds = std::min(a.obs_dim, orl::OBS_PANEL), dcs = std::min(a.critic_obs_dim, orl::OBS_PANEL);
    const size_t smem = wide ? fwdbwd_wide_smem_bytes(ds, dcs) : fwdbwd_smem_bytes(ds, dcs);
    const bool pp = a.obs_dim > orl::OBS_PANEL, pc = a.critic_obs_dim > orl::OBS_PANEL;
    void (*const kern)(OrlPpoArgs) =
        !pp && !pc ? (wide ? ppo_fwdbwd_kernel<orl::MAX_OUT_WIDE, false, false> : ppo_fwdbwd_kernel<orl::MAX_OUT, false, false>)
        : wide ? (pp && pc ? ppo_fwdbwd_kernel<orl::MAX_OUT_WIDE, true, true>
                  : pp ? ppo_fwdbwd_kernel<orl::MAX_OUT_WIDE, true, false> : ppo_fwdbwd_kernel<orl::MAX_OUT_WIDE, false, true>)
               : (pp && pc ? ppo_fwdbwd_kernel<orl::MAX_OUT, true, true>
                  : pp ? ppo_fwdbwd_kernel<orl::MAX_OUT, true, false> : ppo_fwdbwd_kernel<orl::MAX_OUT, false, true>);
    if (a.head_kind == ORL_HEAD_GAUSSIAN_WIDE) {
        void (*const gk)(OrlPpoArgs) = pp && pc ? ppo_fwdbwd_gaussian_wide_kernel<true, true>
                                       : pp ? ppo_fwdbwd_gaussian_wide_kernel<true, false>
                                       : pc ? ppo_fwdbwd_gaussian_wide_kernel<false, true> : ppo_fwdbwd_gaussian_wide_kernel<false, false>;
        const size_t gsmem = fwdbwd_wide_smem_bytes(ds, dcs);
        if (gsmem > 227 * 1024) {
            orl::set_last_error("orl_ppo_fwdbwd: the wide DiagGaussian pass needs %zu bytes of shared memory", gsmem);
            return ORL_ERR_UNSUPPORTED;
        }
        if (int e = orl::allow_dynamic_smem(gk, 227 * 1024)) return e;
        gk<<<2 * a.grid_per_net, P_NT, gsmem, reinterpret_cast<cudaStream_t>(stream)>>>(a);
        ORL_LAUNCH_CHECK("ppo_fwdbwd_gaussian_wide_kernel");
        return 0;
    }
    if (int e = orl::allow_dynamic_smem(kern, 227 * 1024)) return e;
    kern<<<2 * a.grid_per_net, P_NT, smem, reinterpret_cast<cudaStream_t>(stream)>>>(a);
    ORL_LAUNCH_CHECK("ppo_fwdbwd_kernel");
    return 0;
}

extern "C" int orl_ppo_reduce(const OrlPpoArgs* args, void* stream) {
    ORL_CHECK_ARG(args, "args");
    const OrlPpoArgs& a = *args;
    if (int e = check_ppo_args(a)) return e;
    const int stride = orl_ppo_stride(a.obs_dim, a.critic_obs_dim, a.n_actions);
    dim3 grid((stride + 31) / 32, 2);
    ppo_reduce_kernel<<<grid, RED_NT, 0, reinterpret_cast<cudaStream_t>(stream)>>>(a.partials, a.folded, a.grid_per_net, stride);
    ORL_LAUNCH_CHECK("ppo_reduce_kernel");
    return 0;
}

static int check_peer_args(const OrlPeerArgs& pa) {
    ORL_CHECK_ARG(pa.world >= 2 && pa.world <= ORL_PEER_MAX_WORLD && pa.rank >= 0 && pa.rank < pa.world, "peer world / rank");
    ORL_CHECK_ARG(pa.peer_buffers && pa.local_buffer && pa.epochs && pa.error_flag && pa.summed, "null peer buffer");
    ORL_CHECK_ARG(pa.timeout_ms > 0, "timeout_ms");
    return 0;
}

extern "C" long long orl_ppo_peer_bucket_bytes(int obs_dim, int critic_obs_dim, int n_actions, int world) {
    const int stride = orl_ppo_stride(obs_dim, critic_obs_dim, n_actions);
    return (long long)peer_flag_word(world, stride) * sizeof(float) + (long long)3 * ORL_PEER_MAX_WORLD * sizeof(uint32_t) +
           (long long)2 * ORL_PEER_SMALL_MAX * sizeof(double);
}

extern "C" int orl_peer_sum_f64(const OrlPeerArgs* peer, int stride, double* data, int n, void* stream) {
    ORL_CHECK_ARG(peer && data && stride > 0 && stride % 4 == 0, "args");
    if (int e = check_peer_args(*peer)) return e;
    ORL_CHECK_ARG(n > 0 && n <= ORL_PEER_SMALL_MAX, "n must be in 1..ORL_PEER_SMALL_MAX");
    peer_sum_f64_kernel<<<1, 64, 0, reinterpret_cast<cudaStream_t>(stream)>>>(*peer, data, n, stride);
    ORL_LAUNCH_CHECK("peer_sum_f64_kernel");
    return 0;
}

extern "C" int orl_ppo_reduce_peer(const OrlPpoArgs* args, const OrlPeerArgs* peer, void* stream) {
    ORL_CHECK_ARG(args && peer, "args");
    const OrlPpoArgs& a = *args;
    if (int e = check_ppo_args(a)) return e;
    if (int e = check_peer_args(*peer)) return e;
    const int stride = orl_ppo_stride(a.obs_dim, a.critic_obs_dim, a.n_actions);
    dim3 grid((stride + 31) / 32, 2);
    ppo_reduce_peer_kernel<<<grid, RED_NT, 0, reinterpret_cast<cudaStream_t>(stream)>>>(a.partials, *peer, a.grid_per_net, stride);
    ORL_LAUNCH_CHECK("ppo_reduce_kernel(peer)");
    return 0;
}

extern "C" int orl_ppo_apply_peer(const OrlPpoArgs* args, const OrlPeerArgs* peer, void* stream) {
    ORL_CHECK_ARG(args && peer, "args");
    const OrlPpoArgs& a = *args;
    if (int e = check_ppo_args(a)) return e;
    if (int e = check_peer_args(*peer)) return e;
    ORL_CHECK_ARG(a.policy_adam_m && a.policy_adam_v && a.critic_adam_m && a.critic_adam_v && a.adam_steps && a.lrs,
                  "null optimiser state");
    ORL_CHECK_ARG(a.mb_stats, "mb_stats");
    ppo_apply_kernel<true><<<2, 1024, 0, reinterpret_cast<cudaStream_t>(stream)>>>(apply_args(a), *peer);
    ORL_LAUNCH_CHECK("ppo_apply_kernel(peer)");
    return 0;
}

extern "C" int orl_ppo_apply(const OrlPpoArgs* args, void* stream) {
    ORL_CHECK_ARG(args, "args");
    const OrlPpoArgs& a = *args;
    if (int e = check_ppo_args(a)) return e;
    ORL_CHECK_ARG(a.policy_adam_m && a.policy_adam_v && a.critic_adam_m && a.critic_adam_v && a.adam_steps && a.lrs,
                  "null optimiser state");
    ORL_CHECK_ARG(a.mb_stats, "mb_stats");
    ppo_apply_kernel<false><<<2, 1024, 0, reinterpret_cast<cudaStream_t>(stream)>>>(apply_args(a), OrlPeerArgs{});
    ORL_LAUNCH_CHECK("ppo_apply_kernel");
    return 0;
}

extern "C" int orl_minibatch_stats(const int64_t* indices, int64_t batch_rows, const float* returns,
                                   const float* active_masks, double* mb_stats_out, void* stream) {
    ORL_CHECK_ARG(indices && returns && active_masks && mb_stats_out && batch_rows > 0, "null buffer / rows");
    cudaStream_t st = reinterpret_cast<cudaStream_t>(stream);
    int e = orl::check_cuda(cudaMemsetAsync(mb_stats_out, 0, 3 * sizeof(double), st), "memset mb_stats");
    if (e) return e;
    const int grid = (int)std::min<int64_t>((batch_rows + 255) / 256, 4LL * orl::sm_count());
    minibatch_stats_kernel<<<grid, 256, 0, st>>>(indices, batch_rows, returns, active_masks, mb_stats_out);
    ORL_LAUNCH_CHECK("minibatch_stats_kernel");
    return 0;
}
```

### openrl_b200/csrc/orl_ppo_tc.cu

```cuda
#include <cuda.h>

#include <algorithm>
#include <cstdlib>
#include <cstring>
#include <map>
#include <mutex>

#include "orl_loss.cuh"
#include "orl_tc16.cuh"

namespace orl {
int ppo_stride_host(int obs_dim, int critic_obs_dim, int n_actions);
}

namespace {
using namespace orl;
using namespace orl::tc;

constexpr int T_M = 128, T_NT = 256;
constexpr int CW = 32;
constexpr uint32_t PANEL = T_M * 16;
constexpr int R1_PANELS = 10, R2_PANELS = 9, R3_PANELS = 8;
constexpr int P_CST = 8, P_X = 9, P_U = 8;
constexpr int N_LOSS_TC = 8;
constexpr int GA_LD = 84, GB_LD = 20;
constexpr int W3T_LD = 65;
constexpr uint32_t OFF_R1H = 0, OFF_R1L = OFF_R1H + R1_PANELS * PANEL, OFF_R2H = OFF_R1L + R1_PANELS * PANEL,
                   OFF_R2L = OFF_R2H + R2_PANELS * PANEL, OFF_WH = OFF_R2L + R2_PANELS * PANEL, OFF_WL = OFF_WH + 8 * W_PANEL,
                   OFF_R3H = OFF_WL + 8 * W_PANEL, OFF_R3L = OFF_R3H + R3_PANELS * PANEL,
                   OFF_S = OFF_R3L + R3_PANELS * PANEL, OFF_STAGE = OFF_S + T_M * S_LD * 4;
static_assert((T_M * GA_LD + 64 * GB_LD) * 4 <= OFF_WH, "the Ga / Gb staging fits in R1 + R2");
static_assert(OFF_STAGE % 128 == 0, "TMA destination alignment");
static_assert(H * W3T_LD * 4 <= OFF_S - OFF_R3H, "the W3f^T of the flush fits in R3");
static_assert(H * 8 + 6 * H + H * H + MAX_OUT * (H + 1) <= (OFF_S - OFF_R3H) / 4, "the parameter copy of the prologue fits in R3");
static_assert(OFF_R2L + 16 * PANEL <= OFF_R3H, "the 16-panel A descriptors of GEMM3a stop short of R3 (written while they run)");
constexpr int N_SCAL = 4;

struct TcMaps {
    CUtensorMap obs_p, obs_c, actions, old_logp, adv, value_preds, returns, active;
};

__host__ __device__ inline uint32_t tc_stage_bytes(int d) { return (uint32_t)((T_M * d * 4 + 127) & ~127) + N_SCAL * T_M * 4; }
__host__ __device__ inline uint32_t tc_small_off(int d) { return OFF_STAGE + tc_stage_bytes(d); }
constexpr uint32_t SMALL_FLOATS = 8 * H + H + H + MAX_OUT * H + 2 * MAX_OUT;
constexpr uint32_t XCH_FLOATS = MAX_OUT * H + 3 * MAX_OUT + 3 * 8;
__host__ __device__ inline uint32_t tc_smem_bytes(int d) { return tc_small_off(d) + 4 * (SMALL_FLOATS + XCH_FLOATS) + 8; }

constexpr int PH_MAX_CTAS = 1024, PH_WORDS = 9;
#ifdef ORL_PROFILE_PHASES
__device__ unsigned long long g_phases[PH_MAX_CTAS][PH_WORDS];
__device__ __forceinline__ void phase_stamp(int k) {
    if (threadIdx.x != 0 || blockIdx.x >= PH_MAX_CTAS) return;
    unsigned long long t, c;
    unsigned sm;
    asm volatile("mov.u64 %0, %%globaltimer;" : "=l"(t));
    asm volatile("mov.u64 %0, %%clock64;" : "=l"(c));
    asm volatile("mov.u32 %0, %%smid;" : "=r"(sm));
    g_phases[blockIdx.x][k] = t;
    g_phases[blockIdx.x][4 + k] = c;
    g_phases[blockIdx.x][8] = sm;
}
#else
__device__ __forceinline__ void phase_stamp(int) {}
#endif

template <int ACT>
__device__ __forceinline__ float act_bwd_t(float a, bool pos, int activation_id) { return ACT == 1 ? (pos ? 1.f : 0.f) : act_bwd(a, pos, activation_id); }

template <bool POLICY, int NOUT, int ACT, bool TMA>
__device__ __forceinline__ void tc_net_pass(const OrlPpoArgs& a, const TcMaps& maps, uint8_t* smem, int cta, int G, int stride) {
    const int d = POLICY ? a.obs_dim : a.critic_obs_dim;
    const int n = POLICY ? (NOUT == 8 ? a.n_actions : NOUT) : 1;
    const float* params = POLICY ? a.policy_params : a.critic_params;
    const float* obs = POLICY ? a.policy_obs : a.critic_obs;
    const int tid = threadIdx.x, warp = tid >> 5, lane = tid & 31;
    const int row = 16 * warp + (lane & 15), half = lane >> 4, wg = warp >> 2;
    const int cb = CW * half;
    const NetOffsets po = net_offsets(d, n);

    uint8_t* R1h = smem + OFF_R1H; uint8_t* R1l = smem + OFF_R1L;
    uint8_t* R2h = smem + OFF_R2H; uint8_t* R2l = smem + OFF_R2L;
    uint8_t* Wh = smem + OFF_WH;   uint8_t* Wl = smem + OFF_WL;
    uint8_t* R3h = smem + OFF_R3H; uint8_t* R3l = smem + OFF_R3L;
    float* S = reinterpret_cast<float*>(smem + OFF_S);
    float* st_obs = reinterpret_cast<float*>(smem + OFF_STAGE);
    float* st_sc = reinterpret_cast<float*>(smem + OFF_STAGE + ((T_M * d * 4 + 127) & ~127));
    float* w1t = reinterpret_cast<float*>(smem + tc_small_off(d));
    float* b1s = w1t + 8 * H;
    float* b3f = b1s + H;
    float* whf = b3f + H;
    float* bhf = whf + MAX_OUT * H;
    float* swh = bhf + MAX_OUT;
    float* qs = swh + MAX_OUT;
    float* red = qs + MAX_OUT * H + 3 * MAX_OUT;
    uint64_t* bar_st = reinterpret_cast<uint64_t*>(red + 3 * 8);

    const long long n_tiles = (a.batch_rows + T_M - 1) / T_M;
    const float* sc0 = POLICY ? a.actions : a.value_preds;
    const float* sc1 = POLICY ? a.old_log_probs : a.returns;
    const float* sc2 = POLICY ? a.advantages : nullptr;
    const uint32_t stage_tx = (uint32_t)(T_M * d * 4) + (POLICY ? 4u : 3u) * T_M * 4;
    auto issue_tma = [&](long long tile) {
        const int r0 = (int)(a.row_begin + tile * T_M);
        mbar_expect_tx(bar_st, stage_tx);
        tma_load_2d(st_obs, POLICY ? &maps.obs_p : &maps.obs_c, 0, r0, bar_st);
        tma_load_1d(st_sc + 0 * T_M, POLICY ? &maps.actions : &maps.value_preds, r0, bar_st);
        tma_load_1d(st_sc + 1 * T_M, POLICY ? &maps.old_logp : &maps.returns, r0, bar_st);
        if (POLICY) tma_load_1d(st_sc + 2 * T_M, &maps.adv, r0, bar_st);
        tma_load_1d(st_sc + 3 * T_M, &maps.active, r0, bar_st);
    };
    auto issue_gather = [&](long long gi) {
        const bool v = gi >= 0;
        const long long g = v ? gi : 0;
        if (half == 0) {
            if ((d & 3) == 0) {
                for (int k = 0; k < d; k += 4) cp_async16(st_obs + row * d + k, obs + g * d + k, v);
            } else {
                for (int k = 0; k < d; ++k) cp_async4(st_obs + row * d + k, obs + g * d + k, v);
            }
        } else {
            cp_async4(st_sc + 0 * T_M + row, sc0 + g, v);
            cp_async4(st_sc + 1 * T_M + row, sc1 + g, v);
            if (POLICY) cp_async4(st_sc + 2 * T_M + row, sc2 + g, v);
            cp_async4(st_sc + 3 * T_M + row, a.active_masks + g, v);
        }
        cp_async_commit();
    };
    auto row_index = [&](long long tile) -> long long {
        if (tile >= n_tiles) return -1;
        const long long r = tile * T_M + row;
        if (r >= a.batch_rows) return -1;
        return a.indices ? a.indices[r] : a.row_begin + r;
    };
    long long gi_next = -1;
    if (TMA) {
        if (tid == 0) {
            mbar_init(bar_st, 1);
            fence_proxy_async();
            if (cta < n_tiles) { tma_prefetch_desc(POLICY ? &maps.obs_p : &maps.obs_c); issue_tma(cta); }
        }
    } else {
        issue_gather(row_index(cta));
        gi_next = row_index(cta + G);
    }
    long long gi = row_index(cta);

    float* pcopy = reinterpret_cast<float*>(R3h);
    for (int i = tid; i < po.total; i += T_NT) pcopy[i] = params[i];
    const bool pol_masks = a.flags & ORL_PPO_POLICY_ACTIVE_MASKS, val_masks = a.flags & ORL_PPO_VALUE_ACTIVE_MASKS;
    const MbConsts mb = mb_consts(a);
    const double rows_d = loss_rows(a);
    __syncthreads();
    stage_weights_tc(w1t, Wh, Wl, pcopy, d, n, T_NT);
    if (tid >= 4 * 32 && tid < 4 * 32 + MAX_OUT) {
        const int j = tid - 4 * 32;
        float rs = 0.f;
        if (j < n) for (int k = 0; k < H; ++k) rs += folded_wh(pcopy, po, j, k);
        swh[j] = rs;
    }
    if (half == 0) {
        const uint4 z = make_uint4(0u, 0u, 0u, 0u);
        *reinterpret_cast<uint4*>(R1h + P_CST * PANEL + row * 16) = z; *reinterpret_cast<uint4*>(R1l + P_CST * PANEL + row * 16) = z;
        *reinterpret_cast<uint4*>(R1h + P_X * PANEL + row * 16) = z;   *reinterpret_cast<uint4*>(R1l + P_X * PANEL + row * 16) = z;
        *reinterpret_cast<uint4*>(R2h + P_U * PANEL + row * 16) = z;   *reinterpret_cast<uint4*>(R2l + P_U * PANEL + row * 16) = z;
    }
    fence_proxy_async();
    __syncthreads();
    float ga[40], gb[8];
#pragma unroll
    for (int i = 0; i < 40; ++i) ga[i] = 0.f;
#pragma unroll
    for (int i = 0; i < 8; ++i) gb[i] = 0.f;

    float wmax = 0.f;
    for (int i = tid; i < MAX_OUT * H; i += T_NT) wmax = fmaxf(wmax, fabsf(whf[i]));
#pragma unroll
    for (int o = 16; o > 0; o >>= 1) wmax = fmaxf(wmax, __shfl_xor_sync(0xffffffffu, wmax, o));
    if (lane == 0) red[warp] = wmax;
    __syncthreads();
#pragma unroll
    for (int w = 0; w < T_NT / 32; ++w) wmax = fmaxf(wmax, red[w]);
    const double live_d = (POLICY ? pol_masks : val_masks) ? fmin(rows_d, a.mb_stats[2]) : rows_d;
    const int e_rows = (int)ceil(log2(fmax(live_d, 1.0)));
    const int e_u = min(e_rows + 3, 60);
    const int e_z = min(max(e_rows + 3 - (int)floorf(log2f(fmaxf(wmax, 1e-12f))), 0), 60);
    const float Sz = exp2f((float)e_z), Su = exp2f((float)e_u);
    constexpr float SX = 16.f, K1 = 0.25f;
    const float invSz = exp2f(-(float)e_z), invSu = exp2f(-(float)e_u), invS1 = invSz * (1.f / K1);

    const uint64_t dK_A = desc_const(PANEL, 128), dK_W = desc_const(W_PANEL, 128);
    const uint64_t dMN_A = desc_const(128, PANEL), dMN_W = desc_const(128, W_PANEL);
    const uint32_t aR1h = smem_u32(R1h), aR1l = smem_u32(R1l), aR2h = smem_u32(R2h), aR2l = smem_u32(R2l), aWh = smem_u32(Wh), aWl = smem_u32(Wl);
    const uint32_t aR3h = smem_u32(R3h), aR3l = smem_u32(R3l);

    float loss0 = 0.f, loss1 = 0.f, loss2 = 0.f;
    uint32_t it = 0;
    for (long long tile = cta; tile < n_tiles; tile += G, ++it) {
        const uint32_t par = it & 1u;
        if (TMA) mbar_wait(bar_st, par);
        else { cp_async_wait_all(); __syncwarp(); }
        if (it == 0) phase_stamp(1);
        const bool valid = gi >= 0;
        float x[8];
#pragma unroll
        for (int k = 0; k < 8; ++k) x[k] = 0.f;
        if (d == 4) {
            const float4 v = *reinterpret_cast<const float4*>(st_obs + row * 4);
            x[0] = v.x; x[1] = v.y; x[2] = v.z; x[3] = v.w;
        } else {
#pragma unroll
            for (int k = 0; k < 8; ++k) if (k < d) x[k] = st_obs[row * d + k];
        }
        if (!valid) {
#pragma unroll
            for (int k = 0; k < 8; ++k) x[k] = 0.f;
        }
        const float row_a = st_sc[0 * T_M + row], row_b = st_sc[1 * T_M + row];
        const float row_c = POLICY ? st_sc[2 * T_M + row] : 0.f, active = st_sc[3 * T_M + row];

        float n1[CW], s, sq;
        const unsigned posmask = row_fc1<CW, ACT>(x, d, w1t, b1s, cb, a.activation_id, n1, s, sq);
        wgmma_wait<0>();
        row_sum_stats<CW>(s, sq);
        const LnStats l1 = ln_stats(s, sq);

        __syncthreads();
        row_ln1_store<CW>(n1, l1, R1h, R1l, PANEL, row, cb);
        if (half == 0) split_store8(R1h + P_X * PANEL + row * 16, R1l + P_X * PANEL + row * 16, x, SX);
        fence_proxy_async();
        warpgroup_sync(wg);
        float z[32];
#pragma unroll
        for (int i = 0; i < 32; ++i) z[i] = 0.f;
        wgmma_fence();
#pragma unroll
        for (int pass = 0; pass < 3; ++pass) {
            const uint32_t aa = (pass == 0 ? aR1l : aR1h) + wg * 64 * 16, bb = pass == 1 ? aWl : aWh;
#pragma unroll
            for (int kk = 0; kk < 4; ++kk)
                wgmma_f16_n64<0, 0>(z, desc_at(dK_A, aa + 2 * kk * PANEL), desc_at(dK_W, bb + 2 * kk * W_PANEL), (pass | kk) > 0);
        }
        wgmma_commit();
        if (TMA && tid == 0 && tile + G < n_tiles) issue_tma(tile + G);
        long long gi_cur = gi;
        if (!TMA) {
            issue_gather(gi_next);
            gi = gi_next;
            gi_next = row_index(tile + 2 * G);
        } else {
            gi = row_index(tile + G);
        }

        wgmma_wait<0>();
        frag_store<64>(z, S + wg * 64 * S_LD, S_LD);
        __syncwarp();

        float n3[CW], s3, q3;
        row_z3<CW>(S, row, cb, b3f, n3, s3, q3);
        row_sum_stats<CW>(s3, q3);
        const LnStats l3 = ln_stats(s3, q3);
        float out[MAX_OUT];
        row_head<CW, NOUT>(n3, l3, whf, cb, n, out);
        row_sum_head<CW, NOUT>(out, n);
        float dot[MAX_OUT];
#pragma unroll
        for (int j = 0; j < MAX_OUT; ++j) { dot[j] = out[j]; out[j] += (j < NOUT && j < n) ? bhf[j] : 0.f; }

        float dl[MAX_OUT];
#pragma unroll
        for (int j = 0; j < MAX_OUT; ++j) dl[j] = 0.f;
        if (valid) {
            if (POLICY) {
                const float wrow = mb.weight(pol_masks, active);
                const CatRow c = categorical_row<NOUT>(a, out, n, a.action_masks ? a.action_masks + gi_cur * n : nullptr, (int)row_a, row_b,
                                                       apply_adv_norm(mb.adv, row_c), wrow, dl);
                if (half == 0) { loss0 += c.loss * wrow; loss1 += c.ent * wrow; loss2 += c.ratio; }
            } else {
                const float target = (a.flags & ORL_PPO_VALUENORM) ? (row_b - mb.vn_mean) / mb.vn_std : row_b;
                const ValueTerm vt = value_term(out[0], row_a, target, a.clip_param, a.huber_delta, a.flags);
                const float wrow = mb.weight(val_masks, active);
                if (half == 0) loss0 += vt.loss * wrow;
                dl[0] = a.value_loss_coef * wrow * vt.dv;
            }
        }
        float m1 = 0.f, m2 = 0.f;
#pragma unroll
        for (int j = 0; j < MAX_OUT; ++j) dl[j] *= Sz;
        FOR_OUT(j) { m1 = fmaf(dl[j], swh[j], m1); m2 = fmaf(dl[j], dot[j], m2); }
        m1 *= (1.f / H); m2 *= (1.f / H);
#pragma unroll
        for (int q8 = 0; q8 < CW; q8 += 8) {
            float g8[8];
#pragma unroll
            for (int i = 0; i < 8; ++i) g8[i] = 0.f;
#pragma unroll
            for (int q4 = 0; q4 < 8; q4 += 4) {
                FOR_OUT(j) {
                    const float4 wv = *reinterpret_cast<const float4*>(whf + j * H + cb + q8 + q4);
                    g8[q4] = fmaf(dl[j], wv.x, g8[q4]); g8[q4 + 1] = fmaf(dl[j], wv.y, g8[q4 + 1]);
                    g8[q4 + 2] = fmaf(dl[j], wv.z, g8[q4 + 2]); g8[q4 + 3] = fmaf(dl[j], wv.w, g8[q4 + 3]);
                }
            }
#pragma unroll
            for (int i = 0; i < 8; ++i) g8[i] = l3.rstd * (g8[i] - m1 - n3[q8 + i] * m2);
            const uint32_t off = (uint32_t)((cb + q8) >> 3) * PANEL + row * 16;
            split_store8(R2h + off, R2l + off, g8, 1.0f);
        }
        if (half == 0) {
            float u8[8], c8[8];
#pragma unroll
            for (int j = 0; j < 8; ++j) { u8[j] = dl[j] * (l3.rstd * (Su * invSz)); c8[j] = 0.f; }
            c8[0] = 1.0f; c8[1] = l3.mu; c8[2] = l3.var * l3.rstd;
            split_store8(R2h + P_U * PANEL + row * 16, R2l + P_U * PANEL + row * 16, u8, 1.0f);
            split_store8(R1h + P_CST * PANEL + row * 16, R1l + P_CST * PANEL + row * 16, c8, 1.0f);
        }
        fence_proxy_async();
        warpgroup_sync(wg);
#pragma unroll
        for (int i = 0; i < 32; ++i) z[i] = 0.f;
        wgmma_fence();
#pragma unroll
        for (int pass = 0; pass < 3; ++pass) {
            const uint32_t aa = (pass == 0 ? aR2l : aR2h) + wg * 64 * 16, bb = pass == 1 ? aWl : aWh;
#pragma unroll
            for (int kk = 0; kk < 4; ++kk)
                wgmma_f16_n64<0, 1>(z, desc_at(dK_A, aa + 2 * kk * PANEL), desc_at(dMN_W, bb + kk * 256), (pass | kk) > 0);
        }
        wgmma_commit();
        __syncthreads();
#pragma unroll
        for (int pass = 0; pass < 3; ++pass) {
            const uint32_t aa = (pass == 0 ? aR2l : aR2h) + wg * 8 * PANEL, bb = pass == 1 ? aR1l : aR1h;
#pragma unroll
            for (int kk = 0; kk < 8; ++kk)
                wgmma_f16_n80<1, 1>(ga, desc_at(dMN_A, aa + kk * 256), desc_at(dMN_A, bb + kk * 256), 1u);
        }
        wgmma_commit();
        wgmma_wait<1>();
        frag_store<64>(z, S + wg * 64 * S_LD, S_LD);
        __syncwarp();
        {
            float g[CW];
#pragma unroll
            for (int q4 = 0; q4 < CW; q4 += 4) {
                const float4 v = *reinterpret_cast<const float4*>(S + row * S_LD + cb + q4);
                g[q4] = v.x; g[q4 + 1] = v.y; g[q4 + 2] = v.z; g[q4 + 3] = v.w;
            }
            float t1 = 0.f, t2 = 0.f;
#pragma unroll
            for (int i = 0; i < CW; ++i) { t1 += g[i]; t2 = fmaf(g[i], n1[i], t2); }
            row_sum_stats<CW>(t1, t2);
            t1 *= (1.f / H); t2 *= (1.f / H);
            const float std1 = 1.0f / l1.rstd;
#pragma unroll
            for (int i = 0; i < CW; ++i) {
                const float da = l1.rstd * (g[i] - t1 - n1[i] * t2);
                const float aval = fmaf(n1[i], std1, l1.mu);
                g[i] = da * (K1 * act_bwd_t<ACT>(aval, (posmask >> i) & 1u, a.activation_id));
            }
#pragma unroll
            for (int q8 = 0; q8 < CW; q8 += 8) {
                const uint32_t off = (uint32_t)((cb + q8) >> 3) * PANEL + row * 16;
                split_store8(R3h + off, R3l + off, g + q8, 1.0f);
            }
        }
        fence_proxy_async();
        if (wg == 1) {
            asm volatile("bar.sync 3, 256;" ::: "memory");
            wgmma_fence();
#pragma unroll
            for (int pass = 0; pass < 3; ++pass) {
                const uint32_t aa = pass == 0 ? aR3l : aR3h, bb = (pass == 1 ? aR1l : aR1h) + P_CST * PANEL;
#pragma unroll
                for (int kk = 0; kk < 8; ++kk)
                    wgmma_f16_n16<1, 1>(gb, desc_at(dMN_A, aa + kk * 256), desc_at(dMN_A, bb + kk * 256), 1u);
            }
            wgmma_commit();
        } else {
            asm volatile("bar.arrive 3, 256;" ::: "memory");
        }
    }
    wgmma_wait<0>();
    phase_stamp(2);

    float* part = a.partials + (size_t)((POLICY ? 0 : G) + cta) * stride;
    const FoldOffsets fo = fold_offsets(d, n);
    float* qsu = qs + MAX_OUT * H;
    if (it > 0) {
        float* gas = reinterpret_cast<float*>(smem);
        float* gbs = gas + T_M * GA_LD;
        float* w3t = reinterpret_cast<float*>(R3h);
        __syncthreads();
        frag_store<80>(ga, gas + wg * 64 * GA_LD, GA_LD);
        if (wg == 1) frag_store<16>(gb, gbs, GB_LD);
        for (int e = tid; e < H * H; e += T_NT) w3t[(e & 63) * W3T_LD + (e >> 6)] = folded_w3(params, po, e >> 6, e & 63);
        __syncthreads();
        for (int e = tid; e < H * H; e += T_NT) part[fo.g3 + e] = gas[(e >> 6) * GA_LD + (e & 63)] * invSz;
        for (int e = tid; e < n * H; e += T_NT) qs[e] = gas[(H + (e >> 6)) * GA_LD + (e & 63)];
        if (half == 0) {
            const float* c8 = gas + row * GA_LD + 64;
            if (row < H) part[fo.db3 + row] = c8[0] * invSz;
            else if (row < H + n) { qsu[row - H] = c8[0]; qsu[8 + row - H] = c8[1]; qsu[16 + row - H] = c8[2]; }
            if (row < H) {
                const float* g16 = gbs + row * GB_LD;
                part[fo.db1 + row] = g16[0] * invS1;
#pragma unroll
                for (int c = 0; c < 8; ++c) if (c < d) part[fo.g1 + row * d + c] = g16[8 + c] * (invS1 * (1.f / SX));
            }
        }
        __syncthreads();
        for (int o = tid; o < n * H; o += T_NT) {
            const int j = o >> 6, k = o & 63;
            float acc = 0.f;
            for (int i = 0; i < H; ++i) acc = fmaf(qs[j * H + i], w3t[i * W3T_LD + k], acc);
            acc = fmaf(b3f[k], qsu[j], acc) - qsu[8 + j];
            part[fo.gh + o] = acc * invSu;
            if (k == 0) { part[fo.dbh + j] = qsu[16 + j] * invSu; part[fo.dls + j] = 0.f; }
        }
    } else {
        for (int i = tid; i < fo.total; i += T_NT) part[i] = 0.f;
    }
    {
        float v[3] = {loss0, loss1, loss2};
        __syncthreads();
#pragma unroll
        for (int k = 0; k < 3; ++k) { const float sv = warp_sum(v[k]); if (lane == 0) red[k * 8 + warp] = sv; }
        __syncthreads();
        if (tid < N_LOSS_TC) {
            float sv = 0.f;
            if (tid < 3) for (int wv = 0; wv < T_NT / 32; ++wv) sv += red[tid * 8 + wv];
            part[stride - N_LOSS_TC + tid] = sv;
        }
    }
}

template <int NOUT, int ACT, bool TMA>
__global__ void __launch_bounds__(T_NT, 1) ppo_fwdbwd_tc_kernel(const OrlPpoArgs a, const __grid_constant__ TcMaps maps, int stride) {
    extern __shared__ __align__(1024) uint8_t smem_tc[];
    const int G = a.grid_per_net;
    const bool policy = (int)blockIdx.x < G;
    const int cta = policy ? (int)blockIdx.x : (int)blockIdx.x - G;
    phase_stamp(0);
    if (policy) tc_net_pass<true, NOUT, ACT, TMA>(a, maps, smem_tc, cta, G, stride);
    else tc_net_pass<false, 1, ACT, TMA>(a, maps, smem_tc, cta, G, stride);
    phase_stamp(3);
}

using TcKernel = void (*)(const OrlPpoArgs, const TcMaps, int);
template <int NOUT, int ACT>
TcKernel pick_staging(bool tma) { return tma ? ppo_fwdbwd_tc_kernel<NOUT, ACT, true> : ppo_fwdbwd_tc_kernel<NOUT, ACT, false>; }
template <int NOUT>
TcKernel pick_act(int activation_id, bool tma) { return activation_id == 1 ? pick_staging<NOUT, 1>(tma) : pick_staging<NOUT, -1>(tma); }
TcKernel pick_kernel(int n_actions, int activation_id, bool tma) {
    if (n_actions == 2) return pick_act<2>(activation_id, tma);
    if (n_actions == 5) return pick_act<5>(activation_id, tma);
    return pick_act<8>(activation_id, tma);
}

using EncodeTiledFn = CUresult (*)(CUtensorMap*, CUtensorMapDataType, cuuint32_t, void*, const cuuint64_t*, const cuuint64_t*,
                                   const cuuint32_t*, const cuuint32_t*, CUtensorMapInterleave, CUtensorMapSwizzle,
                                   CUtensorMapL2promotion, CUtensorMapFloatOOBfill);
EncodeTiledFn encode_tiled_fn() {
    static EncodeTiledFn fn = nullptr;
    static bool tried = false;
    if (!tried) {
        tried = true;
        void* p = nullptr;
        cudaDriverEntryPointQueryResult q;
        if (cudaGetDriverEntryPoint("cuTensorMapEncodeTiled", &p, cudaEnableDefault, &q) == cudaSuccess && q == cudaDriverEntryPointSuccess)
            fn = reinterpret_cast<EncodeTiledFn>(p);
    }
    return fn;
}
bool make_map_rows(CUtensorMap* m, const float* base, long long rows, int width) {
    EncodeTiledFn fn = encode_tiled_fn();
    if (!fn || !base) return false;
    if (width == 1) {
        cuuint64_t dims[1] = {(cuuint64_t)rows};
        cuuint64_t strides[1] = {0};
        cuuint32_t box[1] = {T_M}, es[1] = {1};
        return fn(m, CU_TENSOR_MAP_DATA_TYPE_FLOAT32, 1, const_cast<float*>(base), dims, strides, box, es, CU_TENSOR_MAP_INTERLEAVE_NONE,
                  CU_TENSOR_MAP_SWIZZLE_NONE, CU_TENSOR_MAP_L2_PROMOTION_NONE, CU_TENSOR_MAP_FLOAT_OOB_FILL_NONE) == CUDA_SUCCESS;
    }
    cuuint64_t dims[2] = {(cuuint64_t)width, (cuuint64_t)rows};
    cuuint64_t strides[1] = {(cuuint64_t)width * 4};
    cuuint32_t box[2] = {(cuuint32_t)width, T_M}, es[2] = {1, 1};
    return fn(m, CU_TENSOR_MAP_DATA_TYPE_FLOAT32, 2, const_cast<float*>(base), dims, strides, box, es, CU_TENSOR_MAP_INTERLEAVE_NONE,
              CU_TENSOR_MAP_SWIZZLE_NONE, CU_TENSOR_MAP_L2_PROMOTION_NONE, CU_TENSOR_MAP_FLOAT_OOB_FILL_NONE) == CUDA_SUCCESS;
}
struct MapKey {
    const void* p[8]; long long rows; int d, dc;
    bool operator<(const MapKey& o) const {
        for (int i = 0; i < 8; ++i) if (p[i] != o.p[i]) return p[i] < o.p[i];
        if (rows != o.rows) return rows < o.rows;
        if (d != o.d) return d < o.d;
        return dc < o.dc;
    }
};
const TcMaps* maps_for(const OrlPpoArgs& a) {
    static std::map<MapKey, TcMaps> cache;
    static std::mutex mu;
    MapKey k{{a.policy_obs, a.critic_obs, a.actions, a.old_log_probs, a.advantages, a.value_preds, a.returns, a.active_masks},
             a.total_rows, a.obs_dim, a.critic_obs_dim};
    std::lock_guard<std::mutex> lock(mu);
    auto it = cache.find(k);
    if (it != cache.end()) return &it->second;
    TcMaps m;
    const bool ok = make_map_rows(&m.obs_p, a.policy_obs, a.total_rows, a.obs_dim) && make_map_rows(&m.obs_c, a.critic_obs, a.total_rows, a.critic_obs_dim) &&
                    make_map_rows(&m.actions, a.actions, a.total_rows, 1) && make_map_rows(&m.old_logp, a.old_log_probs, a.total_rows, 1) &&
                    make_map_rows(&m.adv, a.advantages, a.total_rows, 1) && make_map_rows(&m.value_preds, a.value_preds, a.total_rows, 1) &&
                    make_map_rows(&m.returns, a.returns, a.total_rows, 1) && make_map_rows(&m.active, a.active_masks, a.total_rows, 1);
    if (!ok) return nullptr;
    if (cache.size() > 64) cache.clear();
    return &cache.emplace(k, m).first->second;
}

}

namespace orl {
int launch_ppo_fwdbwd_tc(const OrlPpoArgs& a, cudaStream_t st) {
    if (a.obs_dim > 8 || a.critic_obs_dim > 8) {
        set_last_error("orl_ppo_fwdbwd: ORL_PPO_TENSORCORE supports observation widths <= 8 (got %d / %d)", a.obs_dim, a.critic_obs_dim);
        return ORL_ERR_UNSUPPORTED;
    }
    const int dmax = std::max(a.obs_dim, a.critic_obs_dim);
    const size_t smem = tc_smem_bytes(dmax);
    const int stride = ppo_stride_host(a.obs_dim, a.critic_obs_dim, a.n_actions);
    const bool tma_ok = a.indices == nullptr && (a.obs_dim % 4 == 0) && (a.critic_obs_dim % 4 == 0) &&
                        ((reinterpret_cast<uintptr_t>(a.policy_obs) | reinterpret_cast<uintptr_t>(a.critic_obs) | reinterpret_cast<uintptr_t>(a.actions) |
                          reinterpret_cast<uintptr_t>(a.old_log_probs) | reinterpret_cast<uintptr_t>(a.advantages) | reinterpret_cast<uintptr_t>(a.value_preds) |
                          reinterpret_cast<uintptr_t>(a.returns) | reinterpret_cast<uintptr_t>(a.active_masks)) & 15) == 0 &&
                        a.row_begin + (((a.batch_rows + T_M - 1) / T_M) * T_M) < (1ll << 31);
    const TcMaps* maps = tma_ok ? maps_for(a) : nullptr;
    TcKernel kern = pick_kernel(a.n_actions, a.activation_id, maps != nullptr);
    if (int e = allow_dynamic_smem(kern, tc_smem_bytes(8), true)) return e;
    TcMaps none;
    if (!maps) memset(&none, 0, sizeof(none));
    kern<<<2 * a.grid_per_net, T_NT, smem, st>>>(a, maps ? *maps : none, stride);
    return check_cuda(cudaGetLastError(), "ppo_fwdbwd_tc_kernel");
}
}

#ifdef ORL_PROFILE_PHASES
extern "C" int orl_profile_phases_read(unsigned long long* host) {
    return orl::check_cuda(cudaMemcpyFromSymbol(host, g_phases, sizeof(g_phases)), "orl_profile_phases_read");
}
#endif
```

### openrl_b200/csrc/orl_tc16.cuh

```cuda
#pragma once
#include <cuda_fp16.h>

#include "orl_mlp.cuh"
#include "orl_tc.cuh"

namespace orl {
namespace tc {

constexpr uint32_t W_PANEL = H * 16;

__device__ __forceinline__ uint64_t desc_const(uint32_t lbo_bytes, uint32_t sbo_bytes) {
    return ((uint64_t)((lbo_bytes >> 4) & 0x3FFF) << 16) | ((uint64_t)((sbo_bytes >> 4) & 0x3FFF) << 32);
}
__device__ __forceinline__ uint64_t desc_at(uint64_t dconst, uint32_t smem_addr) { return dconst | (uint64_t)((smem_addr >> 4) & 0x3FFF); }

__device__ __forceinline__ void split2(float a, float b, uint32_t& hi, uint32_t& lo) {
    asm("cvt.rn.satfinite.f16x2.f32 %0, %1, %2;" : "=r"(hi) : "f"(b), "f"(a));
    const __half2 h = *reinterpret_cast<const __half2*>(&hi);
    const float2 hf = __half22float2(h);
    asm("cvt.rn.satfinite.f16x2.f32 %0, %1, %2;" : "=r"(lo) : "f"(b - hf.y), "f"(a - hf.x));
}
__device__ __forceinline__ void split_store8(uint8_t* hi_unit, uint8_t* lo_unit, const float* v, float scale) {
    uint4 h, l;
    split2(v[0] * scale, v[1] * scale, h.x, l.x);
    split2(v[2] * scale, v[3] * scale, h.y, l.y);
    split2(v[4] * scale, v[5] * scale, h.z, l.z);
    split2(v[6] * scale, v[7] * scale, h.w, l.w);
    *reinterpret_cast<uint4*>(hi_unit) = h;
    *reinterpret_cast<uint4*>(lo_unit) = l;
}

__device__ __forceinline__ void stage_weights_tc(float* small, uint8_t* Wh, uint8_t* Wl, const float* __restrict__ params, int d, int n,
                                                 int nt) {
    const int tid = threadIdx.x;
    const NetOffsets po = net_offsets(d, n);
    float* w1t = small; float* b1 = w1t + 8 * H; float* b3f = b1 + H; float* whf = b3f + H; float* bhf = whf + MAX_OUT * H;
    for (int i = tid; i < 8 * H; i += nt) { const int k = i / H, j = i % H; w1t[i] = (k < d) ? params[po.w1 + j * d + k] : 0.f; }
    for (int i = tid; i < H; i += nt) b1[i] = params[po.b1 + i];
    for (int i = tid; i < H * 8; i += nt) {
        const int pnl = i / H, j = i % H;
        float w8[8];
#pragma unroll
        for (int c = 0; c < 8; ++c) w8[c] = folded_w3(params, po, j, 8 * pnl + c);
        const uint32_t off = (uint32_t)pnl * W_PANEL + j * 16;
        split_store8(Wh + off, Wl + off, w8, 1.0f);
    }
    for (int i = tid; i < MAX_OUT * H; i += nt) whf[i] = folded_wh(params, po, i / H, i % H);
    for (int j = tid; j < H; j += nt) b3f[j] = folded_b3(params, po, j);
    for (int j = tid; j < MAX_OUT; j += nt) bhf[j] = folded_bh(params, po, j);
}

constexpr int S_LD = 68;

#define FOR_OUT(j) _Pragma("unroll") for (int j = 0; j < NOUT; ++j) if (NOUT != 8 || j < n)

template <int ACT>
__device__ __forceinline__ float act_tc(float z, int activation_id) { return ACT == 1 ? fmaxf(z, 0.f) : act_fwd(z, activation_id); }

__device__ __forceinline__ void warpgroup_sync(int g) { asm volatile("bar.sync %0, 128;" ::"r"(1 + g) : "memory"); }

template <int CW>
__device__ __forceinline__ void row_sum_stats(float& s, float& sq) {
    if constexpr (CW == 32) {
        s += __shfl_xor_sync(0xffffffffu, s, 16); sq += __shfl_xor_sync(0xffffffffu, sq, 16);
    } else {
        const int qbase = (threadIdx.x & 31) & ~3;
        float ts = 0.f, tq = 0.f;
#pragma unroll
        for (int p = 0; p < 4; ++p) { ts += __shfl_sync(0xffffffffu, s, qbase + p); tq += __shfl_sync(0xffffffffu, sq, qbase + p); }
        s = ts; sq = tq;
    }
}
template <int CW, int NOUT>
__device__ __forceinline__ void row_sum_head(float (&out)[MAX_OUT], int n) {
    if constexpr (CW == 32) {
        FOR_OUT(j) out[j] += __shfl_xor_sync(0xffffffffu, out[j], 16);
    } else {
        const int qbase = (threadIdx.x & 31) & ~3;
        FOR_OUT(j) {
            const float p0 = __shfl_sync(0xffffffffu, out[j], qbase), p1 = __shfl_sync(0xffffffffu, out[j], qbase + 1);
            const float p2 = __shfl_sync(0xffffffffu, out[j], qbase + 2), p3 = __shfl_sync(0xffffffffu, out[j], qbase + 3);
            out[j] = (p0 + p1) + (p2 + p3);
        }
    }
}

struct LnStats {
    float mu, var, rstd;
};
__device__ __forceinline__ LnStats ln_stats(float s, float sq) {
    LnStats l;
    l.mu = s * (1.f / H);
    l.var = fmaxf(sq * (1.f / H) - l.mu * l.mu, 0.f) + LN_EPS;
    l.rstd = 1.0f / sqrtf(l.var);
    return l;
}

template <int CW, int ACT>
__device__ __forceinline__ unsigned row_fc1(const float (&x)[8], int d, const float* w1t, const float* b1s, int cb, int activation_id,
                                            float (&n1)[CW], float& s, float& sq) {
#pragma unroll
    for (int q4 = 0; q4 < CW; q4 += 4) {
        const float4 b = *reinterpret_cast<const float4*>(b1s + cb + q4);
        n1[q4] = b.x; n1[q4 + 1] = b.y; n1[q4 + 2] = b.z; n1[q4 + 3] = b.w;
    }
#pragma unroll
    for (int k = 0; k < 8; ++k) {
        if (k < d) {
#pragma unroll
            for (int q4 = 0; q4 < CW; q4 += 4) {
                const float4 wv = *reinterpret_cast<const float4*>(w1t + k * H + cb + q4);
                n1[q4] = fmaf(x[k], wv.x, n1[q4]); n1[q4 + 1] = fmaf(x[k], wv.y, n1[q4 + 1]);
                n1[q4 + 2] = fmaf(x[k], wv.z, n1[q4 + 2]); n1[q4 + 3] = fmaf(x[k], wv.w, n1[q4 + 3]);
            }
        }
    }
    unsigned posmask = 0u;
    s = 0.f; sq = 0.f;
#pragma unroll
    for (int i = 0; i < CW; ++i) {
        if (n1[i] > 0.f) posmask |= 1u << i;
        n1[i] = act_tc<ACT>(n1[i], activation_id);
        s += n1[i]; sq = fmaf(n1[i], n1[i], sq);
    }
    return posmask;
}

template <int CW>
__device__ __forceinline__ void row_ln1_store(float (&n1)[CW], const LnStats& l, uint8_t* R1h, uint8_t* R1l, uint32_t panel, int row, int cb) {
#pragma unroll
    for (int i = 0; i < CW; ++i) n1[i] = (n1[i] - l.mu) * l.rstd;
#pragma unroll
    for (int q8 = 0; q8 < CW; q8 += 8) {
        const uint32_t off = (uint32_t)((cb + q8) >> 3) * panel + row * 16;
        split_store8(R1h + off, R1l + off, n1 + q8, 1.0f);
    }
}

template <int CW>
__device__ __forceinline__ void row_z3(const float* S, int row, int cb, const float* b3f, float (&n3)[CW], float& s, float& sq) {
#pragma unroll
    for (int q4 = 0; q4 < CW; q4 += 4) {
        const float4 v = *reinterpret_cast<const float4*>(S + row * S_LD + cb + q4);
        n3[q4] = v.x; n3[q4 + 1] = v.y; n3[q4 + 2] = v.z; n3[q4 + 3] = v.w;
    }
    s = 0.f; sq = 0.f;
#pragma unroll
    for (int i = 0; i < CW; ++i) { n3[i] += b3f[cb + i]; s += n3[i]; sq = fmaf(n3[i], n3[i], sq); }
}

template <int CW, int NOUT>
__device__ __forceinline__ void row_head(float (&n3)[CW], const LnStats& l, const float* whf, int cb, int n, float (&out)[MAX_OUT]) {
#pragma unroll
    for (int j = 0; j < MAX_OUT; ++j) out[j] = 0.f;
#pragma unroll
    for (int q4 = 0; q4 < CW; q4 += 4) {
#pragma unroll
        for (int i = 0; i < 4; ++i) n3[q4 + i] = (n3[q4 + i] - l.mu) * l.rstd;
        FOR_OUT(j) {
            const float4 wv = *reinterpret_cast<const float4*>(whf + j * H + cb + q4);
            out[j] = fmaf(n3[q4], wv.x, fmaf(n3[q4 + 1], wv.y, fmaf(n3[q4 + 2], wv.z, fmaf(n3[q4 + 3], wv.w, out[j]))));
        }
    }
}

__device__ __forceinline__ void mbar_expect_tx(uint64_t* bar, uint32_t bytes) {
    asm volatile("mbarrier.arrive.expect_tx.shared::cta.b64 _, [%0], %1;" ::"r"(smem_u32(bar)), "r"(bytes) : "memory");
}
__device__ __forceinline__ void tma_load_1d(void* dst, const void* tmap, int c0, uint64_t* bar) {
    asm volatile("cp.async.bulk.tensor.1d.shared::cluster.global.tile.mbarrier::complete_tx::bytes [%0], [%1, {%2}], [%3];" ::"r"(smem_u32(dst)),
                 "l"(tmap), "r"(c0), "r"(smem_u32(bar))
                 : "memory");
}
__device__ __forceinline__ void tma_load_2d(void* dst, const void* tmap, int c0, int c1, uint64_t* bar) {
    asm volatile("cp.async.bulk.tensor.2d.shared::cluster.global.tile.mbarrier::complete_tx::bytes [%0], [%1, {%2, %3}], [%4];" ::"r"(smem_u32(dst)),
                 "l"(tmap), "r"(c0), "r"(c1), "r"(smem_u32(bar))
                 : "memory");
}
__device__ __forceinline__ void tma_prefetch_desc(const void* tmap) { asm volatile("prefetch.tensormap [%0];" ::"l"(tmap) : "memory"); }

__device__ __forceinline__ void cp_async4(void* dst, const void* src, bool valid) {
    const int sz = valid ? 4 : 0;
    asm volatile("cp.async.ca.shared.global [%0], [%1], 4, %2;" ::"r"(smem_u32(dst)), "l"(src), "r"(sz) : "memory");
}
__device__ __forceinline__ void cp_async16(void* dst, const void* src, bool valid) {
    const int sz = valid ? 16 : 0;
    asm volatile("cp.async.cg.shared.global [%0], [%1], 16, %2;" ::"r"(smem_u32(dst)), "l"(src), "r"(sz) : "memory");
}
__device__ __forceinline__ void cp_async_commit() { asm volatile("cp.async.commit_group;" ::: "memory"); }
__device__ __forceinline__ void cp_async_wait_all() { asm volatile("cp.async.wait_group 0;" ::: "memory"); }

}
}
```

### openrl_b200/lib.py

```python
import ctypes
import os
import re

HERE = os.path.dirname(os.path.abspath(__file__))
LIB_PATH = os.path.join(HERE, "csrc", "libopenrl_b200.so")
HEADER = os.path.join(os.path.dirname(HERE), "include", "openrl_b200.h")


class OrlLibraryError(RuntimeError):
    pass


class OrlError(RuntimeError):
    pass


_c = ctypes
_P = _c.c_void_p
_I = _c.c_int
_D = _c.c_double
_F = _c.c_float
_L = _c.c_longlong

_SIGNATURES = {
    "orl_abi_version": [],
    "orl_device_sm_count": [_c.POINTER(_I)],
    "orl_gae": [_P, _P, _P, _P, _P, _P, _P, _P, _P, _P, _I, _I, _D, _D, _I, _P],
}

_lib = None


def declared_symbols():
    with open(HEADER) as f:
        text = f.read()
    text = re.sub(r"/\*.*?\*/", "", text, flags=re.S)
    return sorted(set(re.findall(r"\b(orl_[a-z0-9_]+)\s*\(", text)))


def load(path=None):
    global _lib
    if _lib is not None and path is None:
        return _lib
    p = path or LIB_PATH
    if not os.path.exists(p):
        raise OrlLibraryError(
            f"{p} not found: build it with `python -m openrl_b200.build` "
            "(nvcc, sm_90a). There is no CPU fallback."
        )
    try:
        lib = ctypes.CDLL(p)
    except OSError as e:
        raise OrlLibraryError(f"cannot load {p}: {e}") from e
    for name, argtypes in _SIGNATURES.items():
        try:
            fn = getattr(lib, name)
        except AttributeError as e:
            raise OrlLibraryError(f"{p} does not export {name}") from e
        fn.argtypes = argtypes
        fn.restype = _I
    lib.orl_last_error.restype = _c.c_char_p
    lib.orl_last_error.argtypes = []
    lib.orl_rnn_workspace_floats.restype = _c.c_int64
    lib.orl_rnn_workspace_floats_for.restype = _c.c_int64
    lib.orl_rnn_workspace_floats_wide_obs.restype = _c.c_int64
    lib.orl_rnn_workspace_floats_head.restype = _c.c_int64
    lib.orl_share_workspace_floats.restype = _c.c_int64
    lib.orl_share_workspace_floats_head.restype = _c.c_int64
    lib.orl_ppo_peer_bucket_bytes.restype = _c.c_int64
    if lib.orl_abi_version() != 1:
        raise OrlLibraryError("ABI version mismatch")
    if path is None:
        _lib = lib
    return lib


def check(code, what=""):
    if code != 0:
        msg = load().orl_last_error().decode(errors="replace")
        raise OrlError(f"{what} failed with code {code}: {msg}")


def ptr(t):
    if t is None:
        return None
    return t.data_ptr()


def current_stream():
    import torch

    return torch.cuda.current_stream().cuda_stream


class OrlRolloutArgs(ctypes.Structure):
    _fields_ = [
        ("env_kind", _c.c_int32), ("n_envs", _c.c_int32), ("n_agents", _c.c_int32), ("episode_length", _c.c_int32),
        ("t_begin", _c.c_int32), ("t_end", _c.c_int32), ("obs_dim", _c.c_int32), ("critic_obs_dim", _c.c_int32),
        ("n_actions", _c.c_int32), ("activation_id", _c.c_int32), ("deterministic", _c.c_int32),
        ("env_table_len", _c.c_int32),
        ("policy_params", _P), ("policy_obs", _P), ("critic_obs", _P), ("actions", _P), ("action_log_probs", _P),
        ("rewards", _P), ("masks", _P), ("active_masks", _P), ("action_masks", _P), ("exp_noise", _P),
        ("rng_seed", _c.c_uint64), ("rng_step_base", _c.c_uint64), ("rng_counter", _P),
        ("env_f64", _P), ("env_u64", _P), ("env_i32", _P), ("env_table", _P),
        ("ep_return", _P), ("ep_length", _P), ("episode_stats", _P),
        ("head_kind", _c.c_int32), ("rng_row_offset", _c.c_int32),
    ]


class OrlSelfPlayArgs(ctypes.Structure):
    _fields_ = [
        ("rollout", OrlRolloutArgs),
        ("pool_params", _P), ("pool_count", _P), ("pool_stats", _P),
        ("pool_capacity", _c.c_int32), ("pool_stride", _c.c_int32), ("strategy", _c.c_int32), ("reserved", _c.c_int32),
    ]


class OrlPpoArgs(ctypes.Structure):
    _fields_ = [
        ("obs_dim", _c.c_int32), ("critic_obs_dim", _c.c_int32), ("n_actions", _c.c_int32),
        ("activation_id", _c.c_int32), ("flags", _c.c_int32), ("grid_per_net", _c.c_int32),
        ("batch_rows", _c.c_int64), ("row_begin", _c.c_int64), ("total_rows", _c.c_int64),
        ("indices", _P),
        ("policy_obs", _P), ("critic_obs", _P), ("actions", _P), ("old_log_probs", _P), ("advantages", _P),
        ("value_preds", _P), ("returns", _P), ("active_masks", _P), ("action_masks", _P),
        ("gae_stats", _P), ("mb_stats", _P), ("vn_state", _P),
        ("policy_params", _P), ("critic_params", _P),
        ("policy_adam_m", _P), ("policy_adam_v", _P), ("critic_adam_m", _P), ("critic_adam_v", _P),
        ("adam_steps", _P), ("lrs", _P),
        ("clip_param", _F), ("entropy_coef", _F), ("value_loss_coef", _F), ("huber_delta", _F), ("max_grad_norm", _F),
        ("adam_beta1", _F), ("adam_beta2", _F), ("adam_eps", _F), ("weight_decay", _F), ("reserved0", _F),
        ("vn_beta", _D),
        ("partials", _P), ("folded", _P), ("grads", _P), ("train_info", _P),
        ("head_kind", _c.c_int32), ("dual_clip_coeff", _F),
        ("norm_rows", _c.c_int64),
    ]


class OrlPeerArgs(ctypes.Structure):
    _fields_ = [
        ("peer_buffers", _P), ("local_buffer", _P), ("epochs", _P), ("error_flag", _P), ("summed", _P),
        ("world", _c.c_int32), ("rank", _c.c_int32), ("timeout_ms", _c.c_int32), ("reserved", _c.c_int32),
    ]


PEER_MAX_WORLD = 16

_SIGNATURES.update({
    "orl_env_reset": [_I, _I, _I, _P, _P, _P, _P, _I, _c.c_uint64, _P, _P, _P],
    "orl_rollout": [_c.POINTER(OrlRolloutArgs), _P],
    "orl_env_step": [_I, _I, _I, _P, _P, _P, _P, _I, _c.c_uint64, _P, _P, _P, _P, _P, _P, _P, _P, _P],
    "orl_critic_values": [_P, _I, _I, _P, _P, _L, _P],
    "orl_selfplay_reset": [_c.POINTER(OrlSelfPlayArgs), _P, _P],
    "orl_selfplay_rollout": [_c.POINTER(OrlSelfPlayArgs), _P],
    "orl_share_param_count": [_I, _I],
    "orl_share_tape_width": [],
    "orl_share_workspace_floats": [_L, _I, _I],
    "orl_share_param_count_head": [_I, _I, _I],
    "orl_share_workspace_floats_head": [_L, _I, _I, _I],
    "orl_share_rollout": [_c.POINTER(OrlRolloutArgs), _P],
    "orl_share_values": [_P, _I, _I, _I, _P, _P, _L, _P],
    "orl_share_fwdbwd": [_c.POINTER(OrlPpoArgs), _P],
    "orl_share_apply": [_c.POINTER(OrlPpoArgs), _P],
    "orl_host_insert": [_P, _I, _I, _I, _P, _P, _P, _P, _P, _I, _P, _I, _P],
    "orl_host_insert_wide_obs": [_P, _I, _I, _I, _P, _P, _P, _P, _P, _I, _P, _I, _P],
    "orl_policy_eval": [_P, _I, _I, _I, _I, _P, _P, _P, _P, _P, _L, _P],
    "orl_ppo_stride": [_I, _I, _I],
    "orl_ppo_grads_stride": [_I, _I, _I],
    "orl_net_param_count": [_I, _I],
    "orl_ppo_fwdbwd": [_c.POINTER(OrlPpoArgs), _P],
    "orl_ppo_reduce": [_c.POINTER(OrlPpoArgs), _P],
    "orl_ppo_apply": [_c.POINTER(OrlPpoArgs), _P],
    "orl_minibatch_stats": [_P, _c.c_int64, _P, _P, _P, _P],
    "orl_ppo_peer_bucket_bytes": [_I, _I, _I, _I],
    "orl_ppo_reduce_peer": [_c.POINTER(OrlPpoArgs), _c.POINTER(OrlPeerArgs), _P],
    "orl_ppo_apply_peer": [_c.POINTER(OrlPpoArgs), _c.POINTER(OrlPeerArgs), _P],
    "orl_peer_sum_f64": [_c.POINTER(OrlPeerArgs), _I, _P, _I, _P],
})


class OrlRnnArgs(ctypes.Structure):
    _fields_ = [
        ("env_kind", _c.c_int32), ("n_envs", _c.c_int32), ("n_agents", _c.c_int32), ("episode_length", _c.c_int32),
        ("t_begin", _c.c_int32), ("t_end", _c.c_int32),
        ("obs_dim", _c.c_int32), ("critic_obs_dim", _c.c_int32), ("n_actions", _c.c_int32), ("activation_id", _c.c_int32),
        ("deterministic", _c.c_int32), ("chunk_length", _c.c_int32),
        ("flags", _c.c_int32), ("env_table_len", _c.c_int32),
        ("n_chunks", _c.c_int64), ("chunk_ids", _P),
        ("policy_params", _P), ("critic_params", _P), ("policy_obs", _P), ("critic_obs", _P),
        ("rnn_states", _P), ("rnn_states_critic", _P),
        ("actions", _P), ("action_log_probs", _P), ("rewards", _P), ("masks", _P), ("active_masks", _P),
        ("value_preds", _P), ("returns", _P), ("advantages", _P), ("exp_noise", _P),
        ("rng_seed", _c.c_uint64), ("rng_step_base", _c.c_uint64), ("rng_counter", _P),
        ("env_f64", _P), ("env_u64", _P), ("env_i32", _P), ("env_table", _P),
        ("ep_return", _P), ("ep_length", _P), ("episode_stats", _P),
        ("gae_stats", _P), ("mb_stats", _P), ("vn_state", _P),
        ("tape", _P), ("grads", _P), ("grads_stride", _c.c_int32), ("reserved1", _c.c_int32),
        ("loss_acc", _P),
        ("policy_adam_m", _P), ("policy_adam_v", _P), ("critic_adam_m", _P), ("critic_adam_v", _P),
        ("adam_steps", _P), ("lrs", _P),
        ("clip_param", _F), ("entropy_coef", _F), ("value_loss_coef", _F), ("huber_delta", _F), ("max_grad_norm", _F),
        ("adam_beta1", _F), ("adam_beta2", _F), ("adam_eps", _F), ("weight_decay", _F), ("dual_clip_coeff", _F),
        ("vn_beta", _D),
        ("train_info", _P),
        ("norm_rows", _c.c_int64),
        ("rng_row_offset", _c.c_int32), ("row_begin", _c.c_int32), ("row_end", _c.c_int32), ("reserved2", _c.c_int32),
        ("action_masks", _P),
        ("head_kind", _c.c_int32), ("reserved3", _c.c_int32),
    ]


_SIGNATURES.update({
    "orl_rnn_act_rows": [_c.POINTER(OrlRnnArgs), _P],
    "orl_host_insert_rnn": [_P, _I, _I, _I, _P, _P, _P, _P, _P, _P, _I, _P, _I, _P],
    "orl_host_insert_rnn_wide": [_P, _I, _I, _I, _P, _P, _P, _P, _P, _P, _I, _P, _I, _P],
    "orl_host_insert_rnn_wide_obs": [_P, _I, _I, _I, _P, _P, _P, _P, _P, _P, _I, _P, _I, _P],
    "orl_rnn_param_count": [_I, _I],
    "orl_rnn_param_count_head": [_I, _I, _I],
    "orl_rnn_tape_width": [],
    "orl_rnn_workspace_floats": [_c.c_int64, _I],
    "orl_rnn_workspace_floats_for": [_c.c_int64, _I, _I],
    "orl_rnn_workspace_floats_wide_obs": [_c.c_int64, _I, _I, _I, _I],
    "orl_rnn_workspace_floats_head": [_c.c_int64, _I, _I, _I, _I, _I],
    "orl_rnn_rollout": [_c.POINTER(OrlRnnArgs), _P],
    "orl_rnn_critic": [_c.POINTER(OrlRnnArgs), _P],
    "orl_rnn_fwdbwd": [_c.POINTER(OrlRnnArgs), _P],
    "orl_rnn_apply": [_c.POINTER(OrlRnnArgs), _P],
})

ENV_NONE, ENV_CARTPOLE, ENV_GRIDWORLD, ENV_MPE_SPREAD, ENV_GRIDWORLD_2P = 0, 1, 2, 3, 4
SP_RANDOM, SP_LAST = 0, 1
HEAD_CATEGORICAL, HEAD_GAUSSIAN = 0, 1
HEAD_GAUSSIAN_WIDE = 2


def is_gaussian(head_kind):
    return head_kind in (HEAD_GAUSSIAN, HEAD_GAUSSIAN_WIDE)
GAE_USE_GAE, GAE_PROPER_TIME_LIMITS, GAE_DENORM = 1, 2, 4
PPO_HUBER, PPO_CLIP_VALUE, PPO_VALUE_ACTIVE_MASKS, PPO_POLICY_ACTIVE_MASKS = 1, 2, 4, 8
PPO_VALUENORM, PPO_ADV_NORMALIZE, PPO_MAX_GRAD_NORM, PPO_TENSORCORE = 16, 32, 64, 128
PPO_TF32 = PPO_TENSORCORE
PPO_A2C, PPO_DUAL_CLIP = 256, 512
PPO_JOINT_ACTION = 1024
```

Before: 241.5 million.

## Precompute folded weight image once per update and bulk-load it; add PDL launches

Each tensor-core fwd/bwd CTA used to copy the raw parameters, fold LayerNorm gains and biases into the weights, split them into fp16 hi/lo panels and compute wmax on its own. That work now happens once, in a fold kernel before the update and again in the Adam apply kernel after each step. It is written to a global weight image that every CTA fetches with one bulk async copy tracked by an mbarrier. The reduce, apply and fwdbwd kernels are also launched with programmatic dependent launch so their prologues can overlap the previous kernel. The cost is extra writes in the apply kernel, more static shared memory there, and a fallback scratch image plus fold launch when no image is supplied.

After: 241.2 million, median of 6. About the same (-0.1%).

```diff
diff --git a/include/openrl_b200.h b/include/openrl_b200.h
--- a/include/openrl_b200.h
+++ b/include/openrl_b200.h
@@ -157,6 +157,7 @@
     int32_t head_kind;
     float dual_clip_coeff;
     int64_t norm_rows;
+    float* weight_image;
 } OrlPpoArgs;
 int orl_ppo_stride(int obs_dim, int critic_obs_dim, int n_actions);
 int orl_ppo_grads_stride(int obs_dim, int critic_obs_dim, int n_actions);
@@ -164,6 +165,8 @@
 int orl_ppo_fwdbwd(const OrlPpoArgs* args, void* stream);
 int orl_ppo_reduce(const OrlPpoArgs* args, void* stream);
 int orl_ppo_apply(const OrlPpoArgs* args, void* stream);
+int orl_ppo_fold(const OrlPpoArgs* args, void* stream);
+int orl_ppo_weight_image_floats(void);
 
 #define ORL_PEER_MAX_WORLD 16
 #define ORL_PEER_SMALL_MAX 16
diff --git a/openrl_b200/algorithms/ppo.py b/openrl_b200/algorithms/ppo.py
--- a/openrl_b200/algorithms/ppo.py
+++ b/openrl_b200/algorithms/ppo.py
@@ -90,6 +90,10 @@
             self.tape = None
             if self.joint_action:
                 self.joint_stats = torch.zeros(6, dtype=torch.float64, device=dev)
+        self.weight_image = None
+        self._image_live = False
+        if self.use_tensor_cores:
+            self.weight_image = torch.empty(int(self._lib.orl_ppo_weight_image_floats()), dtype=torch.float32, device=dev)
         self.gpu_launches = 0
         self.h2d_bytes = 0
         self.d2h_bytes = 0
@@ -137,6 +141,7 @@
         a.action_masks = None if (buf.action_masks_trivial or buf.continuous) else lib.ptr(buf.action_masks)
         a.gae_stats = lib.ptr(buf.gae_stats)
         a.partials, a.folded, a.grads = lib.ptr(self.partials), lib.ptr(self.folded), lib.ptr(self.grads)
+        a.weight_image = lib.ptr(self.weight_image) if self._image_live else None
         return a
 
     def _share_update(self, buf, batch_rows, indices, row_begin, mb_stats):
@@ -293,6 +298,12 @@
         total = buf.episode_length * buf.n_rollout_threads * buf.num_agents
         mb = total // self.num_mini_batch
         whole = self.num_mini_batch == 1
+        if self.weight_image is not None:
+            a = self._common_args(lib.OrlPpoArgs(), mb)
+            a.weight_image = lib.ptr(self.weight_image)
+            lib.check(self._lib.orl_ppo_fold(a, lib.current_stream()), "orl_ppo_fold")
+            self.gpu_launches += 1
+            self._image_live = True
         for _ in range(self.ppo_epoch):
             if self.cfg.parity_mode:
                 perm = torch.randperm(total).to(self.device, non_blocking=True)
@@ -306,3 +317,4 @@
                     self.ppo_update(buf, mb, perm, 0, mb_stats=buf.gae_stats[5:8])
                 else:
                     self.ppo_update(buf, mb, perm[i * mb:(i + 1) * mb])
+        self._image_live = False
diff --git a/openrl_b200/csrc/orl_common.cuh b/openrl_b200/csrc/orl_common.cuh
--- a/openrl_b200/csrc/orl_common.cuh
+++ b/openrl_b200/csrc/orl_common.cuh
@@ -35,6 +35,23 @@
 #define ORL_LAUNCH_CHECK(what) \
     do { int _e = orl::check_cuda(cudaGetLastError(), what); if (_e) return _e; } while (0)
 
+__device__ __forceinline__ void grid_dep_wait() { asm volatile("griddepcontrol.wait;" ::: "memory"); }
+__device__ __forceinline__ void grid_dep_launch() { asm volatile("griddepcontrol.launch_dependents;" ::: "memory"); }
+
+template <typename... KArgs, typename... Args>
+cudaError_t launch_pdl(void (*kernel)(KArgs...), dim3 grid, dim3 block, size_t smem, cudaStream_t st, Args&&... args) {
+    cudaLaunchAttribute attr[1];
+    attr[0].id = cudaLaunchAttributeProgrammaticStreamSerialization;
+    attr[0].val.programmaticStreamSerializationAllowed = 1;
+    cudaLaunchConfig_t cfg = {};
+    cfg.gridDim = grid; cfg.blockDim = block; cfg.dynamicSmemBytes = smem; cfg.stream = st;
+    cfg.attrs = attr; cfg.numAttrs = 1;
+    if (cudaLaunchKernelEx(&cfg, kernel, args...) == cudaSuccess) return cudaSuccess;
+    (void)cudaGetLastError();
+    kernel<<<grid, block, smem, st>>>(args...);
+    return cudaGetLastError();
+}
+
 __device__ __forceinline__ float warp_sum(float v) {
 #pragma unroll
     for (int o = 16; o > 0; o >>= 1) v += __shfl_xor_sync(0xffffffffu, v, o);
diff --git a/openrl_b200/csrc/orl_mlp.cuh b/openrl_b200/csrc/orl_mlp.cuh
--- a/openrl_b200/csrc/orl_mlp.cuh
+++ b/openrl_b200/csrc/orl_mlp.cuh
@@ -56,11 +56,13 @@
     if (i < po.g1) return f[fo.db1 + (i - po.b1)];
     if (i < po.be1) {
         const int k = i - po.g1; float s = 0.f;
+#pragma unroll 16
         for (int j = 0; j < H; ++j) s = fmaf(P[po.w3 + j * H + k], f[fo.g3 + j * H + k], s);
         return s;
     }
     if (i < po.w3) {
         const int k = i - po.be1; float s = 0.f;
+#pragma unroll 16
         for (int j = 0; j < H; ++j) s = fmaf(P[po.w3 + j * H + k], f[fo.db3 + j], s);
         return s;
     }
diff --git a/openrl_b200/csrc/orl_ppo.cu b/openrl_b200/csrc/orl_ppo.cu
--- a/openrl_b200/csrc/orl_ppo.cu
+++ b/openrl_b200/csrc/orl_ppo.cu
@@ -1,6 +1,7 @@
 #include <algorithm>
 
 #include "orl_adam.cuh"
+#include "orl_tc16.cuh"
 
 namespace {
 using namespace orl;
@@ -438,6 +439,8 @@
 __global__ void __launch_bounds__(RED_NT) ppo_reduce_kernel(const float* __restrict__ partials, float* __restrict__ folded, int G, int stride) {
     __shared__ float part[RED_W][32];
     const int net = blockIdx.y, el = blockIdx.x * 32 + (threadIdx.x & 31);
+    grid_dep_wait();
+    grid_dep_launch();
     const float s = reduce_partials(partials, net, G, stride, el, part);
     if (threadIdx.x < 32 && el < stride) folded[(size_t)net * stride + el] = s;
 }
@@ -551,6 +554,8 @@
     float* av = net == 0 ? a.policy_adam_v : a.critic_adam_v;
     float* grads = a.grads + (size_t)net * ppo_grads_stride(a.obs_dim, a.critic_obs_dim, a.n_actions);
     const int tid = threadIdx.x;
+    grid_dep_wait();
+    grid_dep_launch();
     const float* f = PEER ? peer_gather(pa, net, stride) : a.folded + (size_t)net * stride;
 
     float sq = 0.f;
@@ -561,6 +566,10 @@
     }
     const float norm = block_l2_norm(sq);
     adam_step(a, net, params, am, av, grads, po.total, clip_factor(a, norm));
+    if (a.weight_image) {
+        __syncthreads();
+        tc::write_weight_image(reinterpret_cast<uint8_t*>(a.weight_image) + net * tc::IMG_BYTES, params, d, n);
+    }
     if (tid == 0) {
         if (PEER) {
             pa.epochs[net] += 1u;
@@ -622,6 +631,14 @@
     ORL_CHECK_ARG(a.grid_per_net > 0, "grid_per_net");
     ORL_CHECK_ARG(a.batch_rows > 0, "batch_rows");
     ORL_CHECK_ARG(a.policy_params && a.critic_params && a.partials && a.folded && a.grads && a.train_info, "null buffer");
+    return 0;
+}
+
+int check_image_args(const OrlPpoArgs& a) {
+    if (!a.weight_image) return 0;
+    ORL_CHECK_ARG((reinterpret_cast<uintptr_t>(a.weight_image) & 15) == 0, "weight_image must be 16-byte aligned");
+    ORL_CHECK_ARG(a.head_kind == ORL_HEAD_CATEGORICAL && a.obs_dim <= 8 && a.critic_obs_dim <= 8 && a.n_actions <= orl::MAX_OUT,
+                  "weight_image needs a Categorical head, obs dims <= 8 and n_actions <= 8");
     return 0;
 }
 
@@ -698,8 +715,11 @@
     if (int e = check_ppo_args(a)) return e;
     const int stride = orl_ppo_stride(a.obs_dim, a.critic_obs_dim, a.n_actions);
     dim3 grid((stride + 31) / 32, 2);
-    ppo_reduce_kernel<<<grid, RED_NT, 0, reinterpret_cast<cudaStream_t>(stream)>>>(a.partials, a.folded, a.grid_per_net, stride);
-    ORL_LAUNCH_CHECK("ppo_reduce_kernel");
+    const float* partials = a.partials;
+    if (int e = orl::check_cuda(orl::launch_pdl(ppo_reduce_kernel, grid, dim3(RED_NT), 0, reinterpret_cast<cudaStream_t>(stream), partials,
+                                                a.folded, a.grid_per_net, stride),
+                                "ppo_reduce_kernel"))
+        return e;
     return 0;
 }
 
@@ -745,6 +765,7 @@
     ORL_CHECK_ARG(a.policy_adam_m && a.policy_adam_v && a.critic_adam_m && a.critic_adam_v && a.adam_steps && a.lrs,
                   "null optimiser state");
     ORL_CHECK_ARG(a.mb_stats, "mb_stats");
+    if (int e = check_image_args(a)) return e;
     ppo_apply_kernel<true><<<2, 1024, 0, reinterpret_cast<cudaStream_t>(stream)>>>(apply_args(a), *peer);
     ORL_LAUNCH_CHECK("ppo_apply_kernel(peer)");
     return 0;
@@ -757,8 +778,11 @@
     ORL_CHECK_ARG(a.policy_adam_m && a.policy_adam_v && a.critic_adam_m && a.critic_adam_v && a.adam_steps && a.lrs,
                   "null optimiser state");
     ORL_CHECK_ARG(a.mb_stats, "mb_stats");
-    ppo_apply_kernel<false><<<2, 1024, 0, reinterpret_cast<cudaStream_t>(stream)>>>(apply_args(a), OrlPeerArgs{});
-    ORL_LAUNCH_CHECK("ppo_apply_kernel");
+    if (int e = check_image_args(a)) return e;
+    if (int e = orl::check_cuda(orl::launch_pdl(ppo_apply_kernel<false>, dim3(2), dim3(1024), 0, reinterpret_cast<cudaStream_t>(stream),
+                                                apply_args(a), OrlPeerArgs{}),
+                                "ppo_apply_kernel"))
+        return e;
     return 0;
 }
 
diff --git a/openrl_b200/csrc/orl_ppo_tc.cu b/openrl_b200/csrc/orl_ppo_tc.cu
--- a/openrl_b200/csrc/orl_ppo_tc.cu
+++ b/openrl_b200/csrc/orl_ppo_tc.cu
@@ -32,7 +32,7 @@
 static_assert((T_M * GA_LD + 64 * GB_LD) * 4 <= OFF_WH, "the Ga / Gb staging fits in R1 + R2");
 static_assert(OFF_STAGE % 128 == 0, "TMA destination alignment");
 static_assert(H * W3T_LD * 4 <= OFF_S - OFF_R3H, "the W3f^T of the flush fits in R3");
-static_assert(H * 8 + 6 * H + H * H + MAX_OUT * (H + 1) <= (OFF_S - OFF_R3H) / 4, "the parameter copy of the prologue fits in R3");
+static_assert(OFF_WL == OFF_WH + (IMG_WL - IMG_WH), "Wh / Wl as in the weight image: one bulk copy");
 static_assert(OFF_R2L + 16 * PANEL <= OFF_R3H, "the 16-panel A descriptors of GEMM3a stop short of R3 (written while they run)");
 constexpr int N_SCAL = 4;
 
@@ -42,9 +42,8 @@
 
 __host__ __device__ inline uint32_t tc_stage_bytes(int d) { return (uint32_t)((T_M * d * 4 + 127) & ~127) + N_SCAL * T_M * 4; }
 __host__ __device__ inline uint32_t tc_small_off(int d) { return OFF_STAGE + tc_stage_bytes(d); }
-constexpr uint32_t SMALL_FLOATS = 8 * H + H + H + MAX_OUT * H + 2 * MAX_OUT;
 constexpr uint32_t XCH_FLOATS = MAX_OUT * H + 3 * MAX_OUT + 3 * 8;
-__host__ __device__ inline uint32_t tc_smem_bytes(int d) { return tc_small_off(d) + 4 * (SMALL_FLOATS + XCH_FLOATS) + 8; }
+__host__ __device__ inline uint32_t tc_smem_bytes(int d) { return tc_small_off(d) + 4 * (IMG_SMALL_FLOATS + XCH_FLOATS) + 16; }
 
 constexpr int PH_MAX_CTAS = 1024, PH_WORDS = 9;
 #ifdef ORL_PROFILE_PHASES
@@ -90,10 +89,11 @@
     float* b3f = b1s + H;
     float* whf = b3f + H;
     float* bhf = whf + MAX_OUT * H;
-    float* swh = bhf + MAX_OUT;
-    float* qs = swh + MAX_OUT;
+    float* swh = w1t + IMG_SWH;
+    float* qs = w1t + IMG_SMALL_FLOATS;
     float* red = qs + MAX_OUT * H + 3 * MAX_OUT;
     uint64_t* bar_st = reinterpret_cast<uint64_t*>(red + 3 * 8);
+    uint64_t* bar_w = bar_st + 1;
 
     const long long n_tiles = (a.batch_rows + T_M - 1) / T_M;
     const float* sc0 = POLICY ? a.actions : a.value_preds;
@@ -132,32 +132,30 @@
         if (r >= a.batch_rows) return -1;
         return a.indices ? a.indices[r] : a.row_begin + r;
     };
+    if (tid == 0) {
+        mbar_init(bar_st, 1);
+        mbar_init(bar_w, 1);
+        fence_proxy_async();
+        if (TMA && cta < n_tiles) tma_prefetch_desc(POLICY ? &maps.obs_p : &maps.obs_c);
+    }
+    grid_dep_wait();
+    const uint8_t* img = reinterpret_cast<const uint8_t*>(a.weight_image) + (POLICY ? 0 : IMG_BYTES);
     long long gi_next = -1;
     if (TMA) {
-        if (tid == 0) {
-            mbar_init(bar_st, 1);
-            fence_proxy_async();
-            if (cta < n_tiles) { tma_prefetch_desc(POLICY ? &maps.obs_p : &maps.obs_c); issue_tma(cta); }
-        }
+        if (tid == 0 && cta < n_tiles) issue_tma(cta);
     } else {
         issue_gather(row_index(cta));
         gi_next = row_index(cta + G);
     }
+    if (tid == 0) {
+        mbar_expect_tx(bar_w, IMG_BYTES);
+        bulk_load(Wh, img + IMG_WH, IMG_SMALL - IMG_WH, bar_w);
+        bulk_load(w1t, img + IMG_SMALL, IMG_BYTES - IMG_SMALL, bar_w);
+    }
     long long gi = row_index(cta);
-
-    float* pcopy = reinterpret_cast<float*>(R3h);
-    for (int i = tid; i < po.total; i += T_NT) pcopy[i] = params[i];
     const bool pol_masks = a.flags & ORL_PPO_POLICY_ACTIVE_MASKS, val_masks = a.flags & ORL_PPO_VALUE_ACTIVE_MASKS;
     const MbConsts mb = mb_consts(a);
     const double rows_d = loss_rows(a);
-    __syncthreads();
-    stage_weights_tc(w1t, Wh, Wl, pcopy, d, n, T_NT);
-    if (tid >= 4 * 32 && tid < 4 * 32 + MAX_OUT) {
-        const int j = tid - 4 * 32;
-        float rs = 0.f;
-        if (j < n) for (int k = 0; k < H; ++k) rs += folded_wh(pcopy, po, j, k);
-        swh[j] = rs;
-    }
     if (half == 0) {
         const uint4 z = make_uint4(0u, 0u, 0u, 0u);
         *reinterpret_cast<uint4*>(R1h + P_CST * PANEL + row * 16) = z; *reinterpret_cast<uint4*>(R1l + P_CST * PANEL + row * 16) = z;
@@ -172,14 +170,8 @@
 #pragma unroll
     for (int i = 0; i < 8; ++i) gb[i] = 0.f;
 
-    float wmax = 0.f;
-    for (int i = tid; i < MAX_OUT * H; i += T_NT) wmax = fmaxf(wmax, fabsf(whf[i]));
-#pragma unroll
-    for (int o = 16; o > 0; o >>= 1) wmax = fmaxf(wmax, __shfl_xor_sync(0xffffffffu, wmax, o));
-    if (lane == 0) red[warp] = wmax;
-    __syncthreads();
-#pragma unroll
-    for (int w = 0; w < T_NT / 32; ++w) wmax = fmaxf(wmax, red[w]);
+    mbar_wait(bar_w, 0);
+    const float wmax = w1t[IMG_WMAX];
     const double live_d = (POLICY ? pol_masks : val_masks) ? fmin(rows_d, a.mb_stats[2]) : rows_d;
     const int e_rows = (int)ceil(log2(fmax(live_d, 1.0)));
     const int e_u = min(e_rows + 3, 60);
@@ -444,6 +436,33 @@
     if (policy) tc_net_pass<true, NOUT, ACT, TMA>(a, maps, smem_tc, cta, G, stride);
     else tc_net_pass<false, 1, ACT, TMA>(a, maps, smem_tc, cta, G, stride);
     phase_stamp(3);
+}
+
+constexpr int FOLD_NT = 512;
+__global__ void __launch_bounds__(FOLD_NT) ppo_fold_kernel(const float* policy_params, const float* critic_params, float* image, int d,
+                                                           int dc, int n) {
+    grid_dep_wait();
+    grid_dep_launch();
+    const int net = blockIdx.x;
+    write_weight_image(reinterpret_cast<uint8_t*>(image) + net * IMG_BYTES, net == 0 ? policy_params : critic_params, net == 0 ? d : dc,
+                       net == 0 ? n : 1);
+}
+
+int launch_fold(const OrlPpoArgs& a, float* image, cudaStream_t st) {
+    return check_cuda(launch_pdl(ppo_fold_kernel, dim3(2), dim3(FOLD_NT), 0, st, (const float*)a.policy_params, (const float*)a.critic_params,
+                                 image, a.obs_dim, a.critic_obs_dim, a.n_actions),
+                      "ppo_fold_kernel");
+}
+
+float* scratch_image(cudaStream_t st) {
+    static std::map<std::pair<int, cudaStream_t>, float*> images;
+    static std::mutex mu;
+    int dev = 0;
+    if (check_cuda(cudaGetDevice(&dev), "cudaGetDevice")) return nullptr;
+    std::lock_guard<std::mutex> lock(mu);
+    float*& img = images[{dev, st}];
+    if (!img && check_cuda(cudaMalloc(&img, 2 * IMG_BYTES), "cudaMalloc(weight image)")) img = nullptr;
+    return img;
 }
 
 using TcKernel = void (*)(const OrlPpoArgs, const TcMaps, int);
@@ -536,10 +555,28 @@
     if (int e = allow_dynamic_smem(kern, tc_smem_bytes(8), true)) return e;
     TcMaps none;
     if (!maps) memset(&none, 0, sizeof(none));
-    kern<<<2 * a.grid_per_net, T_NT, smem, st>>>(a, maps ? *maps : none, stride);
-    return check_cuda(cudaGetLastError(), "ppo_fwdbwd_tc_kernel");
-}
-}
+    ORL_CHECK_ARG((reinterpret_cast<uintptr_t>(a.weight_image) & 15) == 0, "weight_image must be 16-byte aligned");
+    OrlPpoArgs b = a;
+    if (!b.weight_image) {
+        b.weight_image = scratch_image(st);
+        if (!b.weight_image) return (int)cudaErrorMemoryAllocation;
+        if (int e = launch_fold(b, b.weight_image, st)) return e;
+    }
+    return check_cuda(launch_pdl(kern, dim3(2 * a.grid_per_net), dim3(T_NT), smem, st, b, maps ? *maps : none, stride), "ppo_fwdbwd_tc_kernel");
+}
+}
+
+extern "C" int orl_ppo_fold(const OrlPpoArgs* args, void* stream) {
+    ORL_CHECK_ARG(args, "args");
+    const OrlPpoArgs& a = *args;
+    ORL_CHECK_ARG(a.obs_dim > 0 && a.obs_dim <= 8 && a.critic_obs_dim > 0 && a.critic_obs_dim <= 8, "obs dims must be in 1..8");
+    ORL_CHECK_ARG(a.n_actions > 0 && a.n_actions <= MAX_OUT, "n_actions must be in 1..8");
+    ORL_CHECK_ARG(a.policy_params && a.critic_params, "null buffer");
+    ORL_CHECK_ARG(a.weight_image && (reinterpret_cast<uintptr_t>(a.weight_image) & 15) == 0, "weight_image must be non-null and 16-byte aligned");
+    return launch_fold(a, a.weight_image, reinterpret_cast<cudaStream_t>(stream));
+}
+
+extern "C" int orl_ppo_weight_image_floats() { return 2 * IMG_FLOATS; }
 
 #ifdef ORL_PROFILE_PHASES
 extern "C" int orl_profile_phases_read(unsigned long long* host) {
diff --git a/openrl_b200/csrc/orl_tc16.cuh b/openrl_b200/csrc/orl_tc16.cuh
--- a/openrl_b200/csrc/orl_tc16.cuh
+++ b/openrl_b200/csrc/orl_tc16.cuh
@@ -50,6 +50,82 @@
     for (int j = tid; j < MAX_OUT; j += nt) bhf[j] = folded_bh(params, po, j);
 }
 
+constexpr uint32_t IMG_WH = 0, IMG_WL = IMG_WH + 8 * W_PANEL, IMG_SMALL = IMG_WL + 8 * W_PANEL;
+constexpr int IMG_SWH = 8 * H + H + H + MAX_OUT * H + MAX_OUT;
+constexpr int IMG_WMAX = IMG_SWH + MAX_OUT;
+constexpr int IMG_SMALL_FLOATS = IMG_WMAX + 4;
+constexpr uint32_t IMG_BYTES = IMG_SMALL + 4 * IMG_SMALL_FLOATS;
+constexpr int IMG_FLOATS = (int)IMG_BYTES / 4;
+constexpr int IMG_PARAMS_MAX = 8 * H + 6 * H + H * H + MAX_OUT * (H + 1);
+static_assert(IMG_BYTES % 16 == 0 && (4 * IMG_SMALL_FLOATS) % 16 == 0, "bulk-copy sizes and the second net's image: 16-byte multiples");
+
+constexpr int IMG_LD = H + 1;
+__device__ inline void write_weight_image(uint8_t* img, const float* __restrict__ params, int d, int n) {
+    __shared__ float p[IMG_PARAMS_MAX];
+    __shared__ float w3s[H * IMG_LD], whs[MAX_OUT * IMG_LD];
+    __shared__ float red[32];
+    const int tid = threadIdx.x, nt = blockDim.x, lane = tid & 31;
+    const NetOffsets po = net_offsets(d, n);
+    for (int i = tid; i < po.total; i += nt) p[i] = params[i];
+    for (int i = tid; i < H * H; i += nt) w3s[(i >> 6) * IMG_LD + (i & 63)] = params[po.w3 + i];
+    for (int i = tid; i < MAX_OUT * H; i += nt) whs[(i >> 6) * IMG_LD + (i & 63)] = (i >> 6) < n ? params[po.wh + i] : 0.f;
+    __syncthreads();
+    float* small = reinterpret_cast<float*>(img + IMG_SMALL);
+    float* w1t = small; float* b1 = w1t + 8 * H; float* b3f = b1 + H; float* whf = b3f + H; float* bhf = whf + MAX_OUT * H;
+    const float *g1 = p + po.g1, *be1 = p + po.be1, *g3 = p + po.g3, *be3 = p + po.be3;
+    float wmax = 0.f;
+    if (tid < H) {
+        float s = p[po.b3 + tid];
+#pragma unroll 16
+        for (int k = 0; k < H; ++k) s = fmaf(w3s[tid * IMG_LD + k], be1[k], s);
+        b3f[tid] = s;
+    } else if (tid >= 64 && tid < 64 + MAX_OUT) {
+        const int j = tid - 64;
+        float s = 0.f;
+        if (j < n) {
+            s = p[po.bh + j];
+#pragma unroll 16
+            for (int k = 0; k < H; ++k) s = fmaf(whs[j * IMG_LD + k], be3[k], s);
+        }
+        bhf[j] = s;
+    } else if (tid >= 96 && tid < 96 + MAX_OUT) {
+        const int j = tid - 96;
+        float rs = 0.f;
+        if (j < n) {
+#pragma unroll 16
+            for (int k = 0; k < H; ++k) rs = fmaf(whs[j * IMG_LD + k], g3[k], rs);
+        }
+        small[IMG_SWH + j] = rs;
+    } else if (tid >= 128) {
+        const int t = tid - 128, nw = nt - 128;
+        for (int i = t; i < 8 * H; i += nw) { const int k = i / H, j = i % H; w1t[i] = (k < d) ? p[po.w1 + j * d + k] : 0.f; }
+        for (int i = t; i < H; i += nw) b1[i] = p[po.b1 + i];
+        for (int i = t; i < H * 8; i += nw) {
+            const int pnl = i / H, j = i % H;
+            float w8[8];
+#pragma unroll
+            for (int c = 0; c < 8; ++c) w8[c] = w3s[j * IMG_LD + 8 * pnl + c] * g1[8 * pnl + c];
+            const uint32_t off = (uint32_t)pnl * W_PANEL + j * 16;
+            split_store8(img + IMG_WH + off, img + IMG_WL + off, w8, 1.0f);
+        }
+        for (int i = t; i < MAX_OUT * H; i += nw) {
+            const int j = i / H, k = i % H;
+            const float v = j < n ? whs[j * IMG_LD + k] * g3[k] : 0.f;
+            whf[i] = v;
+            wmax = fmaxf(wmax, fabsf(v));
+        }
+    }
+#pragma unroll
+    for (int o = 16; o > 0; o >>= 1) wmax = fmaxf(wmax, __shfl_xor_sync(0xffffffffu, wmax, o));
+    if (lane == 0) red[tid >> 5] = wmax;
+    __syncthreads();
+    if (tid < 4) {
+        float v = 0.f;
+        if (tid == 0) for (int w = 0; w < nt / 32; ++w) v = fmaxf(v, red[w]);
+        small[IMG_WMAX + tid] = v;
+    }
+}
+
 constexpr int S_LD = 68;
 
 #define FOR_OUT(j) _Pragma("unroll") for (int j = 0; j < NOUT; ++j) if (NOUT != 8 || j < n)
@@ -178,6 +254,11 @@
                  : "memory");
 }
 __device__ __forceinline__ void tma_prefetch_desc(const void* tmap) { asm volatile("prefetch.tensormap [%0];" ::"l"(tmap) : "memory"); }
+__device__ __forceinline__ void bulk_load(void* dst, const void* src, uint32_t bytes, uint64_t* bar) {
+    asm volatile("cp.async.bulk.shared::cluster.global.mbarrier::complete_tx::bytes [%0], [%1], %2, [%3];" ::"r"(smem_u32(dst)),
+                 "l"(src), "r"(bytes), "r"(smem_u32(bar))
+                 : "memory");
+}
 
 __device__ __forceinline__ void cp_async4(void* dst, const void* src, bool valid) {
     const int sz = valid ? 4 : 0;
diff --git a/openrl_b200/lib.py b/openrl_b200/lib.py
--- a/openrl_b200/lib.py
+++ b/openrl_b200/lib.py
@@ -134,6 +134,7 @@
         ("partials", _P), ("folded", _P), ("grads", _P), ("train_info", _P),
         ("head_kind", _c.c_int32), ("dual_clip_coeff", _F),
         ("norm_rows", _c.c_int64),
+        ("weight_image", _P),
     ]
 
 
@@ -171,6 +172,8 @@
     "orl_ppo_fwdbwd": [_c.POINTER(OrlPpoArgs), _P],
     "orl_ppo_reduce": [_c.POINTER(OrlPpoArgs), _P],
     "orl_ppo_apply": [_c.POINTER(OrlPpoArgs), _P],
+    "orl_ppo_fold": [_c.POINTER(OrlPpoArgs), _P],
+    "orl_ppo_weight_image_floats": [],
     "orl_minibatch_stats": [_P, _c.c_int64, _P, _P, _P, _P],
     "orl_ppo_peer_bucket_bytes": [_I, _I, _I, _I],
     "orl_ppo_reduce_peer": [_c.POINTER(OrlPpoArgs), _c.POINTER(OrlPeerArgs), _P],
```
